# yellofi/SelectiveNet_for_semantic_segmentation_binary

Hardware: AMD Instinct MI355X
Metric: train images/sec, SelectiveUNet_B 256x256 bs=128 (global), selective_loss s_lamb=2 (higher is better)
Workload: dtype f32; 1 GPU; SelectiveUNet_B train step, global bs=128, 256x256, Adam lr=1e-3, s_lamb=2; model=SelectiveUNet_B, global_batch=128, per_gpu_batch=128, image=256, parallelism=dp1

## Files before the change

### include/selunet.h

```cpp
#ifndef SELUNET_H
#define SELUNET_H

#include <stdint.h>

#ifdef __cplusplus
extern "C" {
#endif

enum { SELUNET_F32 = 0, SELUNET_BF16 = 1 };

enum {
  SELUNET_OK = 0,
  SELUNET_EINVAL = 1,
  SELUNET_ELAUNCH = 2,
};

enum {
  SELUNET_OPT_HALO = 0,
  SELUNET_OPT_HALO_PERSIST,
  SELUNET_OPT_WINO,
  SELUNET_OPT_WINO_WGRAD,
  SELUNET_OPT_WINO_WGRAD_TW,
  SELUNET_OPT_WINO_WGRAD_WAVES,
  SELUNET_OPT_WGRAD_WGS,
  SELUNET_OPT_X2_WGRAD_WGS,
  SELUNET_OPT_GEMM_WGRAD_WGS,
  SELUNET_OPT_GATHER_WGS,
  SELUNET_OPT_RF_SINGLE,
  SELUNET_OPT_APPLY_U8,
  SELUNET_OPT_APPLY_GRID,
  SELUNET_OPT_X2D,
  SELUNET_OPT_TILE_QUEUE,
  SELUNET_OPT_X2P,
  SELUNET_OPT_CONVT_RING,
  SELUNET_OPT_COUNT
};
int64_t selunet_set_option(int32_t key, int64_t value);

#define SELUNET_GEMM_BM 128

typedef struct selunet_source {
  const void* data;
  const float* scale;
  const float* shift;
  int32_t channels;
  int32_t relu;
  int32_t layout;
  int32_t reserved;
} selunet_source;

typedef struct selunet_gather {
  int32_t n, h, w;
  int32_t taps;
  int32_t nsrc;
  int32_t reserved;
  selunet_source src[2];
} selunet_gather;

enum { SELUNET_EP_PLAIN = 0, SELUNET_EP_SPLIT = 1, SELUNET_EP_SCATTER2X = 2 };

typedef struct selunet_bn_bwd_stats {
  const void* y;
  const float* scale;
  const float* shift;
  const float* mean;
  const float* invstd;
  float* slab;
  float* amax;
} selunet_bn_bwd_stats;

typedef struct selunet_epilogue {
  void* out0;
  void* out1;
  const float* bias;
  float* stats;
  int32_t mode;
  int32_t split;
  float* colsum;
  selunet_bn_bwd_stats bnb;
  float* amax;
  const float* stats_center;
} selunet_epilogue;

const char* selunet_last_error(void);
int32_t selunet_version(void);
const char* selunet_build_id(void);

int selunet_pack_conv3x3(const float* w, int32_t co, int32_t ci, int32_t k_pad, void* fwd,
                         void* dgrad, int32_t dtype, void* stream);
int selunet_pack_convT(const float* w, int32_t ci, int32_t co, void* fwd, void* dgrad,
                       int32_t dtype, void* stream);
int selunet_unpack_conv3x3_grad(const float* packed, int32_t co, int32_t ci, int32_t k_pad,
                                float* out, void* stream);
int selunet_unpack_convT_grad(const float* packed, int32_t ci, int32_t co, float* out, void* stream);

int selunet_gemm_gather(const selunet_gather* a, const void* b, int32_t n_cols, int32_t k_pad,
                        const selunet_epilogue* ep, int32_t dtype, void* stream);
int32_t selunet_conv3x3_wino_ok(int32_t h, int32_t w, int32_t c_in, int32_t c_src0, int32_t n_cols);
int selunet_conv3x3_wino(const selunet_gather* a, const float* u, int32_t n_cols,
                         const selunet_epilogue* ep, void* stream);
const char* selunet_conv3x3_wino_kernel_name(int32_t n_cols, int32_t mode, int32_t split);
int selunet_gemm_gather_x2(const selunet_gather* a, const float* w, int32_t n_cols, int32_t k_pad,
                           const selunet_epilogue* ep, const float* amax0, const float* amax1, void* stream);
int64_t selunet_gemm_gather_x2_stats_rows(const selunet_gather* a, int32_t n_cols);
int64_t selunet_gemm_wgrad_x2_ws_bytes(const selunet_gather* p, const selunet_gather* q);
int selunet_gemm_wgrad_x2(const selunet_gather* p, const selunet_gather* q, float* ws, int64_t ws_bytes, int32_t layout,
                          float* out, const float* amax_p0, const float* amax_p1, const float* amax_q0,
                          const float* amax_q1, void* stream);
int32_t selunet_conv3x3_x2_ok(int32_t h, int32_t w, int32_t c_in, int32_t c_src0, int32_t n_cols);
int64_t selunet_conv3x3_wgrad_x2_ws_bytes(const selunet_gather* p, const selunet_gather* q);
int selunet_conv3x3_wgrad_x2(const selunet_gather* p, const selunet_gather* q, float* ws, int64_t ws_bytes,
                             float* out, const float* amax_p, const float* amax_q0, const float* amax_q1,
                             void* stream);
int selunet_conv3x3_wgrad_x2_bn(const selunet_gather* p, const selunet_gather* q, float* ws, int64_t ws_bytes,
                                float* out, const float* amax_p, const float* amax_q0, const float* amax_q1,
                                const selunet_bn_bwd_stats* bnb, const float* coef, float* dy, float* dy_amax,
                                void* stream);
enum { SELUNET_DA_TENSOR = 0, SELUNET_DA_POOL = 1, SELUNET_DA_HEADS = 2 };
typedef struct selunet_da_source {
  int32_t kind;
  int32_t nh;
  const float* pooled;
  const float* skip;
  const float* head_w;
  const float* g[3];
} selunet_da_source;
int selunet_conv3x3_wgrad_x2_bn_src(const selunet_gather* p, const selunet_gather* q, float* ws, int64_t ws_bytes,
                                    float* out, const float* amax_p, const float* amax_q0, const float* amax_q1,
                                    const selunet_bn_bwd_stats* bnb, const float* coef, const selunet_da_source* src,
                                    float* dy, float* dy_amax, void* stream);
int selunet_conv3x3_x2(const selunet_gather* a, const float* w, int32_t n_cols, const selunet_epilogue* ep,
                       const float* amax0, const float* amax1, void* stream);
const char* selunet_conv3x3_x2_kernel_name(const selunet_gather* a, int32_t n_cols, int32_t mode, int32_t split);
int64_t selunet_conv3x3_x2_stats_rows(const selunet_gather* a, int32_t n_cols);
int selunet_act_bound(const float* gamma, const float* beta, int32_t c, int64_t count, float* out, void* stream);
int selunet_act_amax(const float* y, int64_t m, int32_t c, const float* scale, const float* shift,
                     float* amax, void* stream);
int64_t selunet_gemm_stats_rows(const selunet_gather* a, int32_t n_cols, int32_t dtype);
int32_t selunet_set_halo_workgroups(int32_t wgs);
int32_t selunet_set_gather_workgroups(int32_t wgs);
const char* selunet_gemm_kernel_name(const selunet_gather* a, const selunet_gather* q, int32_t n_cols,
                                     int32_t mode, int32_t dtype);
int selunet_gemm_wgrad(const selunet_gather* p, const selunet_gather* q, float* out,
                       int32_t dtype, void* stream);
int64_t selunet_gemm_wgrad_ws_bytes(const selunet_gather* p, const selunet_gather* q, int32_t dtype);
int selunet_gemm_wgrad_ws(const selunet_gather* p, const selunet_gather* q, float* out, float* ws,
                          int64_t ws_bytes, int32_t dtype, void* stream);
int selunet_gemm_wgrad_ws_to(const selunet_gather* p, const selunet_gather* q, float* packed,
                             float* ws, int64_t ws_bytes, int32_t layout, float* out, int32_t dtype,
                             void* stream);
int32_t selunet_wgrad_ld(int32_t kq);

#define SELUNET_PACK_MAX 32
enum {
  SELUNET_PACK_CONV3X3 = 0,
  SELUNET_PACK_CONVT = 1,
  SELUNET_PACK_CONV3X3_WINO = 2,
  SELUNET_PACK_CONV3X3_X2 = 3,
  SELUNET_PACK_CONVT_X2 = 4,
  SELUNET_PACK_COPY = 5
};
typedef struct selunet_pack_desc {
  const float* w;
  void* fwd;
  void* dgrad;
  int32_t kind, co, ci, k_pad;
  int64_t offset;
} selunet_pack_desc;
typedef struct selunet_pack_list {
  int32_t n, _pad;
  selunet_pack_desc d[SELUNET_PACK_MAX];
} selunet_pack_list;
int selunet_pack_weights(const selunet_pack_list* list, int32_t dtype, void* stream);

int64_t selunet_reduce_ws_bytes(int32_t cols);
int selunet_reduce_rows(const float* slab, int64_t rows, int32_t cols, double* ws, double* out,
                        float* out32, void* stream);
int64_t selunet_channel_slab_rows(int64_t m);
int selunet_channel_sum(const void* x, int64_t m, int32_t c, float* slab, int32_t dtype, void* stream);

int selunet_bn_finalize(const double* sums, int64_t count, int32_t c, const float* conv_bias,
                        const float* gamma, const float* beta, float* running_mean,
                        float* running_var, int64_t* num_batches, float momentum, float eps,
                        int32_t training, float* mean, float* invstd, float* scale, float* shift,
                        void* stream);
int selunet_bn_bwd_reduce(const void* dz, const void* y, int64_t m, int32_t c, const float* scale,
                          const float* shift, const float* mean, const float* invstd, float* slab,
                          int32_t dtype, void* stream);
int selunet_bn_bwd_finalize(const double* sums, int64_t count, int32_t c, const float* gamma,
                            const float* invstd, float* dgamma, float* dbeta, float* dbias,
                            float* coef, void* stream);
int selunet_bn_stats_finalize(const float* slab, int64_t rows, double* ws, double* sums, int64_t count,
                              int32_t c, const float* conv_bias, const float* gamma, const float* beta,
                              float* running_mean, float* running_var, int64_t* num_batches,
                              float momentum, float eps, float* mean, float* invstd, float* scale,
                              float* shift, void* stream);
int64_t selunet_bn_centered_rows(int64_t m);
int selunet_bn_centered_partials(const void* y, int64_t m, int32_t c, const float* center, float* slab,
                                 int32_t dtype, void* stream);
int selunet_bn_centered_partials_adaptive(const void* y, int64_t m, int32_t c, const float* center,
                                          const float* uvar, float ratio, float* slab, int32_t dtype,
                                          void* stream);
int selunet_bn_stats_finalize_shifted(const float* slab, int64_t rows, double* ws, int64_t count, int32_t c,
                                      float* center, const float* conv_bias, const float* gamma,
                                      const float* beta, float ratio, float* mean, float* uvar_flag,
                                      float* invstd, float* scale, float* shift, void* stream);
int selunet_bn_stats_finalize_centered(const float* slab, int64_t rows, double* ws, double* sums,
                                       int64_t count, int32_t c, const float* center,
                                       const float* conv_bias, const float* gamma, const float* beta,
                                       float* running_mean, float* running_var, int64_t* num_batches,
                                       float momentum, float eps, float* mean, float* invstd,
                                       float* scale, float* shift, void* stream);
int selunet_bn_stats_finalize_centered_bound(const float* slab, int64_t rows, double* ws, double* sums,
// ... 204 lines not shown
```

### selectivenet_for_semantic_segmentation_binary_amd/_lib.py

```python
from __future__ import annotations

import ctypes
import os
import threading

import torch

from . import build as _build

c_int32, c_int64, c_double, c_float, c_void_p = (ctypes.c_int32, ctypes.c_int64, ctypes.c_double,
                                                ctypes.c_float, ctypes.c_void_p)

F32, BF16 = 0, 1
EP_PLAIN, EP_SPLIT, EP_SCATTER2X = 0, 1, 2
DA_TENSOR, DA_POOL, DA_HEADS = 0, 1, 2
GEMM_BM = 128
ADAM_CHUNK = 4096
SWEEP_MAX = 256
AUC_CHUNK = 4096


class Source(ctypes.Structure):
    _fields_ = [("data", c_void_p), ("scale", c_void_p), ("shift", c_void_p), ("channels", c_int32),
                ("relu", c_int32), ("layout", c_int32), ("reserved", c_int32)]


class Gather(ctypes.Structure):
    _fields_ = [("n", c_int32), ("h", c_int32), ("w", c_int32), ("taps", c_int32), ("nsrc", c_int32),
                ("reserved", c_int32), ("src", Source * 2)]


class BnBwdStats(ctypes.Structure):
    _fields_ = [("y", c_void_p), ("scale", c_void_p), ("shift", c_void_p), ("mean", c_void_p),
                ("invstd", c_void_p), ("slab", c_void_p), ("amax", c_void_p)]


class DaSource(ctypes.Structure):
    _fields_ = [("kind", c_int32), ("nh", c_int32), ("pooled", c_void_p), ("skip", c_void_p), ("head_w", c_void_p),
                ("g", c_void_p * 3)]


class Epilogue(ctypes.Structure):
    _fields_ = [("out0", c_void_p), ("out1", c_void_p), ("bias", c_void_p), ("stats", c_void_p),
                ("mode", c_int32), ("split", c_int32), ("colsum", c_void_p), ("bnb", BnBwdStats),
                ("amax", c_void_p), ("stats_center", c_void_p)]


class PackDesc(ctypes.Structure):
    _fields_ = [("w", c_void_p), ("fwd", c_void_p), ("dgrad", c_void_p), ("kind", c_int32), ("co", c_int32),
                ("ci", c_int32), ("k_pad", c_int32), ("offset", c_int64)]


PACK_MAX, PACK_CONV3X3, PACK_CONVT, PACK_CONV3X3_WINO, PACK_CONV3X3_X2, PACK_CONVT_X2, PACK_COPY = 32, 0, 1, 2, 3, 4, 5
WG_CONV3X3, WG_CONVT = 1, 2


class PackList(ctypes.Structure):
    _fields_ = [("n", c_int32), ("_pad", c_int32), ("d", PackDesc * PACK_MAX)]


class HeadPlanes(ctypes.Structure):
    _fields_ = [("n", c_int32), ("hw", c_int32), ("plane", c_void_p * 8), ("img_stride", c_int64 * 8),
                ("w_off", c_int32 * 8), ("b_off", c_int32 * 8), ("row_len", c_int32)]


class AdamTensor(ctypes.Structure):
    _fields_ = [("param", c_void_p), ("grad", c_void_p), ("exp_avg", c_void_p), ("exp_avg_sq", c_void_p),
                ("numel", c_int64), ("chunk_begin", c_int64)]


P = c_void_p
SIGNATURES = {
    "selunet_last_error": (ctypes.c_char_p, []),
    "selunet_version": (c_int32, []),
    "selunet_build_id": (ctypes.c_char_p, []),
    "selunet_pack_conv3x3": (c_int32, [P, c_int32, c_int32, c_int32, P, P, c_int32, P]),
    "selunet_pack_convT": (c_int32, [P, c_int32, c_int32, P, P, c_int32, P]),
    "selunet_unpack_conv3x3_grad": (c_int32, [P, c_int32, c_int32, c_int32, P, P]),
    "selunet_unpack_convT_grad": (c_int32, [P, c_int32, c_int32, P, P]),
    "selunet_gemm_gather": (c_int32, [ctypes.POINTER(Gather), P, c_int32, c_int32, ctypes.POINTER(Epilogue),
                                      c_int32, P]),
    "selunet_gemm_wgrad": (c_int32, [ctypes.POINTER(Gather), ctypes.POINTER(Gather), P, c_int32, P]),
    "selunet_wgrad_ld": (c_int32, [c_int32]),
    "selunet_gemm_wgrad_ws_bytes": (c_int64, [ctypes.POINTER(Gather), ctypes.POINTER(Gather), c_int32]),
    "selunet_gemm_wgrad_ws": (c_int32, [ctypes.POINTER(Gather), ctypes.POINTER(Gather), P, P, c_int64, c_int32, P]),
    "selunet_gemm_wgrad_ws_to": (c_int32, [ctypes.POINTER(Gather), ctypes.POINTER(Gather), P, P, c_int64, c_int32, P,
                                           c_int32, P]),
    "selunet_conv3x3_wino_ok": (c_int32, [c_int32, c_int32, c_int32, c_int32, c_int32]),
    "selunet_conv3x3_wino": (c_int32, [ctypes.POINTER(Gather), P, c_int32, ctypes.POINTER(Epilogue), P]),
    "selunet_conv3x3_wino_kernel_name": (ctypes.c_char_p, [c_int32, c_int32, c_int32]),
    "selunet_conv3x3_x2_ok": (c_int32, [c_int32, c_int32, c_int32, c_int32, c_int32]),
    "selunet_gemm_gather_x2": (c_int32, [ctypes.POINTER(Gather), P, c_int32, c_int32, ctypes.POINTER(Epilogue), P, P,
                                         P]),
    "selunet_conv3x3_x2": (c_int32, [ctypes.POINTER(Gather), P, c_int32, ctypes.POINTER(Epilogue), P, P, P]),
    "selunet_conv3x3_x2_kernel_name": (ctypes.c_char_p, [ctypes.POINTER(Gather), c_int32, c_int32, c_int32]),
    "selunet_conv3x3_x2_stats_rows": (c_int64, [ctypes.POINTER(Gather), c_int32]),
    "selunet_act_bound": (c_int32, [P, P, c_int32, c_int64, P, P]),
    "selunet_act_amax": (c_int32, [P, c_int64, c_int32, P, P, P, P]),
    "selunet_conv3x3_wgrad_x2_ws_bytes": (c_int64, [ctypes.POINTER(Gather), ctypes.POINTER(Gather)]),
    "selunet_gemm_wgrad_x2_ws_bytes": (c_int64, [ctypes.POINTER(Gather), ctypes.POINTER(Gather)]),
    "selunet_gemm_wgrad_x2": (c_int32, [ctypes.POINTER(Gather), ctypes.POINTER(Gather), P, c_int64, c_int32, P, P, P,
                                        P, P, P]),
    "selunet_conv3x3_wgrad_x2": (c_int32, [ctypes.POINTER(Gather), ctypes.POINTER(Gather), P, c_int64, P, P, P, P,
                                           P]),
    "selunet_conv3x3_wgrad_x2_bn": (c_int32, [ctypes.POINTER(Gather), ctypes.POINTER(Gather), P, c_int64, P, P, P, P,
                                              ctypes.POINTER(BnBwdStats), P, P, P, P]),
    "selunet_conv3x3_wgrad_x2_bn_src": (c_int32, [ctypes.POINTER(Gather), ctypes.POINTER(Gather), P, c_int64, P, P, P,
                                                  P, ctypes.POINTER(BnBwdStats), P, ctypes.POINTER(DaSource), P, P,
                                                  P]),
    "selunet_gemm_stats_rows": (c_int64, [ctypes.POINTER(Gather), c_int32, c_int32]),
    "selunet_gemm_gather_x2_stats_rows": (c_int64, [ctypes.POINTER(Gather), c_int32]),
    "selunet_set_halo_workgroups": (c_int32, [c_int32]),
    "selunet_set_gather_workgroups": (c_int32, [c_int32]),
    "selunet_gemm_kernel_name": (ctypes.c_char_p, [ctypes.POINTER(Gather), ctypes.POINTER(Gather), c_int32, c_int32,
                                                   c_int32]),
    "selunet_reduce_ws_bytes": (c_int64, [c_int32]),
    "selunet_reduce_rows": (c_int32, [P, c_int64, c_int32, P, P, P, P]),
    "selunet_channel_slab_rows": (c_int64, [c_int64]),
    "selunet_bn_centered_rows": (c_int64, [c_int64]),
    "selunet_channel_sum": (c_int32, [P, c_int64, c_int32, P, c_int32, P]),
    "selunet_bn_finalize": (c_int32, [P, c_int64, c_int32, P, P, P, P, P, P, c_float, c_float, c_int32, P, P, P, P,
                                      P]),
    "selunet_bn_bwd_reduce": (c_int32, [P, P, c_int64, c_int32, P, P, P, P, P, c_int32, P]),
    "selunet_bn_bwd_finalize": (c_int32, [P, c_int64, c_int32, P, P, P, P, P, P, P]),
    "selunet_pack_weights": (c_int32, [ctypes.POINTER(PackList), c_int32, P]),
    "selunet_bn_stats_finalize": (c_int32, [P, c_int64, P, P, c_int64, c_int32, P, P, P, P, P, P, c_float, c_float,
                                            P, P, P, P, P]),
    "selunet_bn_centered_partials": (c_int32, [P, c_int64, c_int32, P, P, c_int32, P]),
    "selunet_bn_centered_partials_adaptive": (c_int32, [P, c_int64, c_int32, P, P, c_float, P, c_int32, P]),
    "selunet_bn_stats_finalize_centered": (c_int32, [P, c_int64, P, P, c_int64, c_int32, P, P, P, P, P, P, P,
                                                     c_float, c_float, P, P, P, P, P]),
    "selunet_bn_stats_finalize_centered_bound": (c_int32, [P, c_int64, P, P, c_int64, c_int32, P, P, P, P, P, P, P,
                                                           c_float, c_float, P, P, P, P, P, P]),
    "selunet_bn_bwd_stats_finalize": (c_int32, [P, c_int64, P, P, c_int64, c_int32, P, P, P, P, P, P, P]),
    "selunet_bn_bwd_stats_finalize_bound": (c_int32, [P, c_int64, P, P, c_int64, c_int32, P, P, P, P, P, P, P, P, P]),
    "selunet_bn_bwd_apply": (c_int32, [P, P, c_int64, c_int32, P, P, P, P, P, P, c_int32, P]),
    "selunet_bn_bwd_apply_amax": (c_int32, [P, P, c_int64, c_int32, P, P, P, P, P, P, P, c_int32, P]),
    "selunet_bn_bwd_apply_heads": (c_int32, [P, c_int64, P, P, P, P, P, P, c_int32, P, P, P, P, P, c_int32, P]),
    "selunet_bn_bwd_apply_heads_planes": (c_int32, [P, c_int64, P, P, P, P, P, P, ctypes.POINTER(HeadPlanes), P, P,
                                                    c_int32, P]),
    "selunet_bn_bwd_apply_pool": (c_int32, [P, c_int32, c_int32, c_int32, c_int32, P, P, P, P, P, P, P, P, P,
                                            c_int32, P]),
    "selunet_im2col3x3": (c_int32, [P, c_int32, c_int32, c_int32, c_int32, c_int32, P, c_int32, P]),
    "selunet_maxpool2_fwd": (c_int32, [P, c_int32, c_int32, c_int32, c_int32, P, P, P, c_int32, P]),
    "selunet_maxpool2_bwd": (c_int32, [P, c_int32, c_int32, c_int32, c_int32, P, P, P, P, P,
                                       ctypes.POINTER(BnBwdStats), c_int32, P]),
    "selunet_maxpool2_bwd_slab_rows": (c_int64, [c_int32, c_int32, c_int32, c_int32]),
    "selunet_first_conv_rows": (c_int64, [c_int32, c_int32, c_int32]),
    "selunet_first_conv_fwd": (c_int32, [P, c_int32, c_int32, c_int32, c_int32, P, P, P, c_int32, P]),
    "selunet_first_conv_fwd_centered": (c_int32, [P, c_int32, c_int32, c_int32, c_int32, P, P, P, P, c_int32, P]),
    "selunet_bn_stats_finalize_shifted": (c_int32, [P, c_int64, P, c_int64, c_int32, P, P, P, P, c_float, P, P, P, P,
                                                    P, P]),
    "selunet_first_conv_wgrad_rows": (c_int64, [c_int32, c_int32, c_int32]),
    "selunet_first_conv_wgrad": (c_int32, [P, c_int32, c_int32, c_int32, c_int32, P, P, c_int32, P]),
    "selunet_first_conv_wgrad_bn": (c_int32, [P, c_int32, c_int32, c_int32, c_int32, P, P, P, P, P, P, P, P, c_int32,
                                              P]),
    "selunet_heads_fwd": (c_int32, [P, c_int64, P, P, P, P, c_int32, P, P, P, c_int32, P]),
    "selunet_heads_bwd": (c_int32, [P, c_int64, P, P, P, c_int32, P, P, P, P, P, ctypes.POINTER(BnBwdStats),
                                    c_int32, P]),
    "selunet_heads_fwd_planes": (c_int32, [P, c_int64, P, P, P, P, ctypes.POINTER(HeadPlanes), c_int32, P]),
    "selunet_heads_bwd_planes": (c_int32, [P, c_int64, P, P, P, ctypes.POINTER(HeadPlanes), P, P,
                                           ctypes.POINTER(BnBwdStats), c_int32, P]),
    "selunet_ce_selective_partials": (c_int32, [P, P, P, c_int64, c_int32, c_int64, P, P]),
    "selunet_ce_selective_bwd": (c_int32, [P, P, P, c_int64, c_int32, c_int64, P, c_float, P, P, P, P, P]),
    "selunet_ce_selective_partials_hard": (c_int32, [P, P, P, c_int64, c_int32, c_int64, P, P]),
    "selunet_ce_selective_bwd_hard": (c_int32, [P, P, P, c_int64, c_int32, c_int64, P, P, P, P, P]),
    "selunet_ce_partials": (c_int32, [P, P, c_int64, c_int32, c_int64, P, P]),
    "selunet_ce_bwd": (c_int32, [P, P, c_int64, c_int32, c_int64, c_double, P, P, P]),
    "selunet_loss_slab_rows": (c_int64, [c_int64]),
    "selunet_selective_partials": (c_int32, [P, P, P, c_int64, P, P]),
    "selunet_selective_finalize": (c_int32, [P, c_double, c_float, c_float, P, P, P, P]),
    "selunet_selective_bwd": (c_int32, [P, P, P, c_int64, P, c_float, P, P, P, P, P]),
    "selunet_selective_partials_hard": (c_int32, [P, P, P, c_int64, P, P]),
    "selunet_selective_bwd_hard": (c_int32, [P, P, P, c_int64, P, P, P, P, P]),
    "selunet_bce_partials": (c_int32, [P, P, c_int64, P, P]),
    "selunet_bce_finalize": (c_int32, [P, c_double, P, P]),
    "selunet_bce_bwd": (c_int32, [P, P, c_int64, c_double, P, P, P]),
    "selunet_adam_step": (c_int32, [P, c_int32, c_int64, c_float, c_float, c_float, c_float, c_float, c_int64, P]),
    "selunet_memset": (c_int32, [P, c_int32, c_int64, P]),
    "selunet_memcpy": (c_int32, [P, P, c_int64, P]),
    "selunet_stream_create": (c_int32, [ctypes.POINTER(P)]),
    "selunet_stream_destroy": (c_int32, [P]),
    "selunet_graph_capture_begin": (c_int32, [P]),
    "selunet_graph_capture_end": (c_int32, [P, ctypes.POINTER(P)]),
    "selunet_graph_launch": (c_int32, [P, P]),
    "selunet_graph_destroy": (c_int32, [P]),
    "selunet_prep_batch": (c_int32, [P, P, P, c_int32, c_int32, c_int32, c_int32, P, P, P]),
    "selunet_prep_batch_mode": (c_int32, [P, P, P, c_int32, c_int32, c_int32, c_int32, P, P, P]),
    "selunet_seg_metrics": (c_int32, [P, P, P, c_int64, c_float, c_float, P, P]),
    "selunet_seg_metrics_sweep": (c_int32, [P, P, P, c_int64, c_float, P, c_int32, P, P]),
    "selunet_seg_metrics_rows": (c_int32, [P, P, P, c_int32, c_int64, c_float, c_float, P, P]),
    "selunet_patch_auc": (c_int32, [P, P, P, c_int32, c_int64, c_float, P, P]),
    "selunet_tile_gather": (c_int32, [P, c_int32, c_int32, P, c_int32, c_int32, c_int32, c_int32, P, P]),
    "selunet_tile_stitch": (c_int32, [P, P, P, c_int32, c_int32, c_int32, c_int32, c_int32, c_int32, c_int32, c_int32,
                                      c_float, c_float, P, P, P, P, P, P]),
    "selunet_tile_gather_flip": (c_int32, [P, c_int32, c_int32, P, c_int32, c_int32, c_int32, c_int32, c_int32, P, P]),
    "selunet_image_transpose": (c_int32, [P, c_int32, c_int32, P, P]),
    "selunet_tta_accumulate": (c_int32, [P, P, P] + [c_int32] * 9 + [c_float, c_float, P, P, P, P, P]),
    "selunet_tta_finalize": (c_int32, [P] * 8 + [c_int32] * 5 + [c_float, c_float] + [P] * 8),
    "selunet_regions_label": (c_int32, [P, c_int64, c_int32, c_int32, c_int32, c_int32, P, P, P, c_int32, P, c_int32,
                                        P]),
    "selunet_regions_stats": (c_int32, [P, c_int32, P, c_int64, P, c_int64, c_int32, c_int32, P, c_int32, c_int64, P,
                                        P]),
    "selunet_regions_apply": (c_int32, [P, c_int64, c_int32, c_int32, P, c_int32, P, c_int32, P, c_int64, P, P]),
    "selunet_tissue_plane": (c_int32, [P, c_int32, c_int32, c_int32, c_int32, P, c_int32, P]),
    "selunet_tile_tissue_counts": (c_int32, [P, c_int64, c_int32, c_int32, P, c_int32, c_int32, c_int32, c_int32, P, P]),
    "selunet_tissue_class_counts": (c_int32, [P, c_int64, P, c_int64, c_int32, c_int32, P, P]),
    "selunet_set_option": (c_int64, [c_int32, c_int64]),
    "selunet_cu_hold": (c_int32, [P, P, c_int64, c_int32, c_float, P]),
}

_lib = None
_lock = threading.Lock()


def lib_path() -> str:
    return os.environ.get("SELUNET_LIB", _build.LIB)


def load(auto_build: bool = False):
    global _lib
    if _lib is not None:
        return _lib
    with _lock:
        if _lib is not None:
            return _lib
        path = lib_path()
        tree = _build.source_fingerprint()
        own = "SELUNET_LIB" not in os.environ
        if auto_build and own and (not os.path.exists(path) or _build.lib_stamp(path) != _build.build_id(tree)):
            _build.build(verbose=False)
        if not os.path.exists(path):
            raise RuntimeError(
                f"{path} not found: the MI355X kernels are not built (run "
                "`python -m selectivenet_for_semantic_segmentation_binary_amd.build`). "
                "There is no CPU fallback.")
        L = ctypes.CDLL(path)
        L.selunet_build_id.restype = ctypes.c_char_p
        built_fp, built_arch = _build.parse_build_id(L.selunet_build_id().decode())
        if own and built_fp != tree:
            raise RuntimeError(
                f"{path} was built from other sources (build id {built_fp}, for {built_arch}; tree "
                f"{tree}): rebuild with `python -m selectivenet_for_semantic_segmentation_binary_amd.build`")
        for name, (res, args) in SIGNATURES.items():
            fn = getattr(L, name)
            fn.restype = res
            fn.argtypes = args
        _lib = L
        for env, key in ENV_OPTIONS.items():
            v = os.environ.get(env)
            if v is not None and v.strip().lstrip("-").isdigit():
                L.selunet_set_option(key, int(v))
        if os.environ.get("SELUNET_NO_HALO") == "1":
            L.selunet_set_option(OPT["HALO"], 0)
    return _lib


OPT = {name: i for i, name in enumerate([
    "HALO", "HALO_PERSIST", "WINO", "WINO_WGRAD", "WINO_WGRAD_TW", "WINO_WGRAD_WAVES", "WGRAD_WGS",
    "X2_WGRAD_WGS", "GEMM_WGRAD_WGS", "GATHER_WGS", "RF_SINGLE", "APPLY_U8", "APPLY_GRID", "X2D",
    "TILE_QUEUE", "X2P", "CONVT_RING"])}
ENV_OPTIONS = {f"SELUNET_{k}": v for k, v in OPT.items() if k != "HALO"}


def set_option(name: str, value: int) -> int:
    return int(load().selunet_set_option(OPT[name], int(value)))


class SelunetError(RuntimeError):
    pass


_HOOK = None


def set_call_hook(hook):
    global _HOOK
    _HOOK = hook


def call(name, *args):
    L = load()
    fn = getattr(L, name)
    if _REC is not None:
        _REC.record(name, fn, args)
    rc = fn(*args) if _HOOK is None else _HOOK(name, args, lambda: fn(*args))
    if rc != 0:
        raise SelunetError(f"{name}: {L.selunet_last_error().decode()}")
    return rc


class Slot:
    __slots__ = ("name", "offset")

    def __init__(self, name, offset):
        self.name, self.offset = name, offset


class Plan:

    MAX_GRAPHS = 4

    def __init__(self, slots):
        self._ranges = [(n, t.data_ptr(), t.data_ptr() + t.numel() * t.element_size()) for n, t in slots.items()
                        if t is not None]
        self.calls = []
        self.keep = []
        self.stream = stream_ptr()
        self._graphs = {}
        self._seen = set()
        self._graphable = graphs_enabled()

    def _slot(self, v):
        if isinstance(v, int) and v:
            for n, lo, hi in self._ranges:
                if lo <= v < hi:
                    return Slot(n, v - lo)
        return None

    def record(self, name, fn, args):
        args = list(args)
        pos = []
        for i, a in enumerate(args):
            if isinstance(a, ctypes.Structure):
                fields = _struct_slots(a, self._slot)
                if fields:
                    args[i] = _StructSlots(type(a).from_buffer_copy(a), fields)
                    pos.append(i)
                continue
            sl = self._slot(a)
            if sl is not None:
                args[i] = sl
                pos.append(i)
        self.calls.append((name, fn, tuple(args), tuple(pos)))

    def record_marker(self, tag):
        self.calls.append((None, None, tag, ()))

    def _bound(self, base):
        for name, fn, args, pos in self.calls:
            if pos:
                a = list(args)
                for i in pos:
                    a[i] = a[i].bind(base) if isinstance(a[i], _StructSlots) else base[a[i].name] + a[i].offset
# ... 241 lines not shown
```

### selectivenet_for_semantic_segmentation_binary_amd/csrc/conv3x3.hip

```cpp
#include <cstdlib>

#include "gemm_common.h"

namespace selunet {

constexpr int TH = 16, TW = 16;
constexpr int HHT = TH + 2, HWT = TW + 2;
constexpr int HPIX = HHT * HWT;
constexpr int HTHREADS = 512;
constexpr int A_ROUNDS = (HPIX * 8 + HTHREADS - 1) / HTHREADS;
constexpr int AROWB = 160;
__device__ __forceinline__ int halo_off(int hp, int cc) { return hp * AROWB + ((cc ^ ((hp / HWT) & 1)) << 4); }

template <typename T, int BN, bool ONE_CHUNK>
__global__ void __launch_bounds__(HTHREADS, ONE_CHUNK ? 2 : 1)
conv3x3_halo_kernel(GatherArg g, const T* __restrict__ B, int N, int k_pad, EpiArg ep, int n_tiles, int tiles_x,
                    int tiles_y) {
  constexpr int E = 16 / sizeof(T);
  constexpr int CK = 128 / sizeof(T);
  constexpr int WAVES_N = BN / 64;
  constexpr int WAVES_M = 8 / WAVES_N;
  constexpr int WPIX = (TH * TW) / WAVES_M;
  constexpr int MT = WPIX / 32;
  constexpr int NT = 2;
// ... 133 lines not shown
  b_store(rb_next, 0);
  rb_next = b_load(nsteps > 1 ? 1 : 0);
  __syncthreads();

  if constexpr (ONE_CHUNK) {
#pragma unroll
    for (int t = 0; t < 9; ++t) {
      BRegs rb_far = rb_next;
      if (t + 2 < 9) rb_far = b_load(t + 2);
      mma_step(0, t & 1, t);
      if (t + 1 < 9) b_store(rb_next, (t + 1) & 1);
      __syncthreads();
      rb_next = rb_far;
    }
  } else {
    uint4 ra[A_ROUNDS];
    for (int c = 0; c < nchunks; ++c) {
      const int cn = c + 1 < nchunks ? c + 1 : c;
      int cs = cn * CK;
      const bool s1 = g.nsrc > 1 && cs >= g.src[0].C;
      if (s1) cs -= g.src[0].C;
      const SrcArg sn = pick_src(g, s1 ? 1 : 0);
      float* ssc = Ss + ((c + 1) & 1) * CK;
      float* ssh = Ss + 2 * CK + ((c + 1) & 1) * CK;
      float coef = 0.0f;
#pragma unroll
      for (int t = 0; t < 9; ++t) {
        const int s = c * 9 + t;
        const BRegs rb_far = b_load(s + 2 < nsteps ? s + 2 : nsteps - 1);
        if (t == 0 && sn.scale && tid < 2 * CK) coef = tid < CK ? sn.scale[cs + tid] : sn.shift[cs + tid - CK];
        if (t < A_ROUNDS) {
          int hp, cc;
          a_slot(t, hp, cc);
          ra[t] = *a_ptr(cn, hp, cc);
        }
        mma_step(c & 1, s & 1, t);
        b_store(rb_next, (s + 1) & 1);
        if (t == 1 && sn.scale && tid < 2 * CK) (tid < CK ? ssc[tid] : ssh[tid - CK]) = coef;
        if (t >= AD && t - AD < A_ROUNDS) {
          const int r = t - AD;
          int hp, cc;
          if (a_slot(r, hp, cc)) {
            uint4 v = make_uint4(0, 0, 0, 0);
            if (a_inside(hp)) {
              v = ra[r];
              if (sn.scale) {
                T e[E];
                __builtin_memcpy(e, &v, 16);
#pragma unroll
                for (int j = 0; j < E; ++j) {
                  float f = to_f(e[j]) * ssc[cc * E + j] + ssh[cc * E + j];
                  if (sn.relu) f = fmaxf(f, 0.0f);
                  e[j] = from_f<T>(f);
                }
                __builtin_memcpy(&v, e, 16);
              }
            }
            *reinterpret_cast<uint4*>(As + ((c + 1) & 1) * HPIX * AROWB + halo_off(hp, cc)) = v;
          }
        }
        __syncthreads();
        rb_next = rb_far;
      }
    }
  }

  float* tile = reinterpret_cast<float*>(smem);
  acc_to_lds<MT, NT, BN>(tile, acc, wm * WPIX, wn * 64, lane);
  __syncthreads();
  auto dst = [&](int pix, int c) -> T* {
    const int y = y0 + pix / TW, x = x0 + pix % TW;
    if (y >= g.h || x >= g.w) return nullptr;
    const int64_t m = ((int64_t)img * g.h + y) * g.w + x;
    const int col = n0 + c;
    if (ep.mode == SELUNET_EP_SPLIT)
      return col < ep.split ? reinterpret_cast<T*>(ep.out0) + m * ep.split + col
                            : reinterpret_cast<T*>(ep.out1) + m * (N - ep.split) + (col - ep.split);
    return reinterpret_cast<T*>(ep.out0) + m * N + col;
  };
  auto bias_col = [&](int c) { return n0 + c; };
  lds_tile_store<T, TH * TW, BN, HTHREADS>(tile, tid, dst, ep.bias, bias_col, tile_stats(ep, ptile, n0, N));
}

template <typename T, int BN, bool X2, bool M16 = false, bool TQ = false>
__global__ void __launch_bounds__(HTHREADS, 1)
conv3x3_halo_persist_kernel(GatherArg g, const T* __restrict__ B, int N, int k_pad, EpiArg ep, int n_tiles,
                            int tiles_x, int tiles_y, int ptiles, int gp, const float* __restrict__ wcs,
                            const float* __restrict__ amax0, const float* __restrict__ amax1,
                            unsigned* __restrict__ tq = nullptr) {
  static_assert(!TQ || X2, "tile queue: split-fp16 kernel only");
  static_assert(!X2 || std::is_same<T, float>::value, "split-fp16 form of fp32 operands only");
  static_assert(!M16 || X2, "16x16x32 form: split-fp16 only (the bf16 form lost every A/B, retired in round 6)");
  constexpr int E = 16 / sizeof(T);
  constexpr int CK = 128 / sizeof(T);
  constexpr int WAVES_N = BN / 64;
  constexpr int WAVES_M = 8 / WAVES_N;
  constexpr int WPIX = (TH * TW) / WAVES_M;
  constexpr int MT = WPIX / 32;
  constexpr int NT = 2;
  constexpr int RT = WPIX / 16;
  using AccT = std::conditional_t<M16, f32x4, f32x16>;
  constexpr int AM = M16 ? RT : MT, AN = M16 ? 4 : NT;
  constexpr int WROWB = M16 ? 160 : ROWB;
  constexpr int B_ROUNDS = BN * 8 / HTHREADS;
  static_assert(B_ROUNDS * HTHREADS == BN * 8, "weight tile rows must split evenly over the threads");
  auto halo_load_tap = [](int r) { return r; };
  auto halo_write_tap = [](int r) { return r + 3; };
  static_assert(A_ROUNDS <= 6, "halo slice schedule covers six slices");

  constexpr int SMEM_MAIN = 2 * HPIX * AROWB + 2 * BN * WROWB + 2 * CK * 8;
  constexpr int SMEM_EPI = TH * TW * (BN + 4) * 4;
  __shared__ __attribute__((aligned(16))) unsigned char smem[SMEM_MAIN > SMEM_EPI ? SMEM_MAIN : SMEM_EPI];
  unsigned char* As = smem;
  unsigned char* Bs = smem + 2 * HPIX * AROWB;
  float* Ss = reinterpret_cast<float*>(Bs + 2 * BN * WROWB);

  const int tid = threadIdx.x;
  const int lane = tid & 63, wave = tid >> 6;
  const int wm = wave / WAVES_N, wn = wave % WAVES_N;
  const int half = lane >> 5, l32 = lane & 31;
  const int l16 = lane & 15, kg = lane >> 4;

  const unsigned lb = xcd_remap(blockIdx.x, gridDim.x);
  const int n_tile = lb % n_tiles;
  const int prow = lb / n_tiles;
  const int n0 = n_tile * BN;
  const int nchunks = g.Ctot / CK;
  const int ntl = TQ ? 0 : (prow < ptiles ? (ptiles - prow + gp - 1) / gp : 0);
  __shared__ int tq_slot;
  int pt_cur = 0, pt_next = 0;
  if constexpr (TQ) {
    if (tid == 0) tq_slot = (int)min(atomicAdd(tq + n_tile, 1u), (unsigned)ptiles);
    __syncthreads();
    pt_cur = tq_slot;
  }
  const int csteps = nchunks * 9;
  float xs = 1.0f;
  float cfac[AN] = {};
  if constexpr (X2) {
    float am = amax0 ? amax0[0] : 0.0f;
    if (g.nsrc > 1 && amax1) am = fmaxf(am, amax1[0]);
    float inv;
    xs = x2_scale(am, &inv);
#pragma unroll
    for (int b = 0; b < AN; ++b)
      cfac[b] = wcs[n0 + wn * 64 + (M16 ? b * 16 + l16 : b * 32 + l32)] * inv;
  }
  auto halo_store = [&](int hb, int hp, int cc, uint4 v) __attribute__((always_inline)) {
    unsigned char* base = As + hb * HPIX * AROWB + hp * AROWB;
    if constexpr (X2) {
      float f[4];
      __builtin_memcpy(f, &v, 16);
      f16x4 h, l;
#pragma unroll
      for (int e = 0; e < 4; ++e) {
        _Float16 a, b;
        x2_split(f[e] * xs, a, b);
        h[e] = a;
        l[e] = b;
      }
      const int par = (hp / HWT) & 1;
      *reinterpret_cast<f16x4*>(base + (((cc >> 1) ^ par) << 4) + (cc & 1) * 8) = h;
      *reinterpret_cast<f16x4*>(base + (((4 + (cc >> 1)) ^ par) << 4) + (cc & 1) * 8) = l;
    } else {
      *reinterpret_cast<uint4*>(base + (((cc ^ ((hp / HWT) & 1))) << 4)) = v;
    }
  };

  auto halo_store_prepped = [&](int hb, int hp, int cc, uint4 v) __attribute__((always_inline)) {
    unsigned char* base = As + hb * HPIX * AROWB + hp * AROWB;
    if constexpr (X2) {
      const int par = (hp / HWT) & 1;
      *reinterpret_cast<uint2*>(base + (((cc >> 1) ^ par) << 4) + (cc & 1) * 8) = make_uint2(v.x, v.y);
      *reinterpret_cast<uint2*>(base + (((4 + (cc >> 1)) ^ par) << 4) + (cc & 1) * 8) = make_uint2(v.z, v.w);
// ... 368 lines not shown
            if (!defer) x_put((J + 1) & 1, r, xlds, o);
            else ra[r] = o;
            continue;
          }
          int hp, cc;
          if (a_slot(r, hp, cc)) {
            uint4 v = make_uint4(0, 0, 0, 0);
            if (a_inside(ny0, nx0, hp)) {
              v = ra[r];
              if (sn.scale) {
                T e[E];
                __builtin_memcpy(e, &v, 16);
#pragma unroll
                for (int j = 0; j < E; ++j) {
                  float f = to_f(e[j]) * ssc[cc * E + j] + ssh[cc * E + j];
                  if (sn.relu) f = fmaxf(f, 0.0f);
                  e[j] = from_f<T>(f);
                }
                __builtin_memcpy(&v, e, 16);
              }
            }
            if (!defer) {
              halo_store((J + 1) & 1, hp, cc, v);
            } else {
              if constexpr (X2) {
                float f[4];
                __builtin_memcpy(f, &v, 16);
                f16x4 h, l;
#pragma unroll
                for (int e = 0; e < 4; ++e) {
                  _Float16 a, b;
                  x2_split(f[e] * xs, a, b);
                  h[e] = a;
                  l[e] = b;
                }
                __builtin_memcpy(&v.x, &h, 8);
                __builtin_memcpy(&v.z, &l, 8);
              }
              ra[r] = v;
            }
          }
        }
        __syncthreads();
        rb_next = rb_far;
        ++S;
      }
      if (defer) {
      }
    }

    if constexpr (X2) {
#pragma unroll
      for (int a = 0; a < AM; ++a)
#pragma unroll
        for (int b = 0; b < AN; ++b) acc[a][b] *= cfac[b];
    }
    if constexpr (M16) {
#pragma unroll
      for (int a = 0; a < RT; ++a)
#pragma unroll
        for (int b = 0; b < 4; ++b)
#pragma unroll
          for (int i = 0; i < 4; ++i)
            tile[(wm * WPIX + a * 16 + 4 * kg + i) * (BN + 4) + wn * 64 + b * 16 + l16] = acc[a][b][i];
    } else {
      acc_to_lds<MT, NT, BN>(tile, acc, wm * WPIX, wn * 64, lane);
    }
#pragma unroll
    for (int a = 0; a < AM; ++a)
#pragma unroll
      for (int b = 0; b < AN; ++b) acc[a][b] = AccT{};
    __syncthreads();
    auto dst = [&](int pix, int cl) -> T* {
      const int y = y0 + pix / TW, x = x0 + pix % TW;
      if (y >= g.h || x >= g.w) return nullptr;
      const int64_t m = ((int64_t)img * g.h + y) * g.w + x;
      const int col = n0 + cl;
      if (ep.mode == SELUNET_EP_SPLIT)
        return col < ep.split ? reinterpret_cast<T*>(ep.out0) + m * ep.split + col
                              : reinterpret_cast<T*>(ep.out1) + m * (N - ep.split) + (col - ep.split);
      return reinterpret_cast<T*>(ep.out0) + m * N + col;
    };
    auto bias_col = [&](int cl) { return n0 + cl; };
    if constexpr (TQ) {
      TileStats tt = tile_stats(ep, pt_cur, n0, N);
      lds_tile_store_acc<T, TH * TW, BN, HTHREADS>(tile, tid, dst, ep.bias, bias_col, tt, s1, s2, s3, amx);
      tt.amax = nullptr;
      tile_stats_flush<BN, HTHREADS>(tile, tid, tt, s1, s2, s3, 0.0f);
#pragma unroll
      for (int e = 0; e < 8; ++e) s1[e] = s2[e] = s3[e] = 0;
    } else {
      lds_tile_store_acc<T, TH * TW, BN, HTHREADS>(tile, tid, dst, ep.bias, bias_col, ts, s1, s2, s3, amx);
    }
    if (TQ ? pt_next < ptiles : i + 1 < ntl) {
      __syncthreads();
      int tid2 = tid;
      asm volatile("" : "+v"(tid2));
#pragma unroll
      for (int r = 0; r < A_ROUNDS; ++r) {
        if constexpr (X2) {
          x_put(J & 1, r, x_lds(tid2), ra[r]);
        } else {
          const int hidx = r * HTHREADS + tid2;
          if (hidx < HPIX * 8) halo_store_prepped(J & 1, hidx >> 3, hidx & 7, ra[r]);
        }
      }
      b_store(rb_hold, S & 1);
      __syncthreads();
    }
    if constexpr (TQ) pt_cur = pt_next;
    gc = gn;
  }
  if constexpr (TQ) {
    if (ts.amax) block_amax(ts.amax, amx, tile);
    if (tid == 0 && atomicAdd(tq + n_tiles + n_tile, 1u) == (unsigned)gp - 1u) {
      atomicExch(tq + n_tile, 0u);
      atomicExch(tq + n_tiles + n_tile, 0u);
    }
  } else {
    tile_stats_flush<BN, HTHREADS>(tile, tid, ts, s1, s2, s3, amx);
  }
}

constexpr int WINO_STEPS = 12;
__device__ __forceinline__ int wino_row(int hp) {
  const int hy = hp / HWT, hx = hp - hy * HWT;
  return hy * HWT + (hx & 1) * (HWT / 2) + (hx >> 1);
}

template <int BN, int XS>
__global__ void __launch_bounds__(HTHREADS, 1)
conv3x3_wino_persist_kernel(GatherArg g, const float* __restrict__ B, int N, int k_pad, EpiArg ep, int n_tiles,
                            int tiles_x, int tiles_y, int ptiles, int gp) {
  using T = float;
  constexpr int E = 4;
  constexpr int CK = 32;
  constexpr int NT = BN / 64;
  constexpr int STEPS = WINO_STEPS / XS;
  constexpr int BROWS = XS * BN;
  constexpr int B_ROUNDS = BROWS * 8 / HTHREADS;
  static_assert(XS == 1 || XS == 2, "one or two planes per step");
  auto lt = [](int r) { return XS == 1 ? r : r >> 1; };
  static_assert(B_ROUNDS * HTHREADS == BROWS * 8, "weight tile rows must split evenly over the threads");
  static_assert(A_ROUNDS <= 6, "halo slice schedule covers six slices");

  constexpr int SMEM_MAIN = 2 * HPIX * AROWB + 2 * BROWS * ROWB + 2 * CK * 8;
  constexpr int SMEM_EPI = TH * TW * (BN + 4) * 4;
  __shared__ __attribute__((aligned(16))) unsigned char smem[SMEM_MAIN > SMEM_EPI ? SMEM_MAIN : SMEM_EPI];
  unsigned char* As = smem;
  unsigned char* Bs = smem + 2 * HPIX * AROWB;
  float* Ss = reinterpret_cast<float*>(Bs + 2 * BROWS * ROWB);

  const int tid = threadIdx.x;
  const int lane = tid & 63, wave = tid >> 6;
  const int wm = wave >> 1, wn = wave & 1;
  const int half = lane >> 5, l32 = lane & 31;
  const int pair = wm * 32 + l32, py = pair >> 3, px2 = pair & 7;

  const unsigned lb = xcd_remap(blockIdx.x, gridDim.x);
  const int n_tile = lb % n_tiles;
  const int prow = lb / n_tiles;
  const int n0 = n_tile * BN;
  const int ntl = prow < ptiles ? (ptiles - prow + gp - 1) / gp : 0;
  const int nchunks = g.Ctot / CK;
  const int csteps = nchunks * STEPS;

  auto tile_xy = [&](int i, int& img, int& y0, int& x0) __attribute__((always_inline)) {
    const unsigned pt = (unsigned)(prow + i * gp);
    const unsigned r = pt / (unsigned)tiles_x;
    x0 = (int)(pt - r * (unsigned)tiles_x) * TW;
    const unsigned r2 = r / (unsigned)tiles_y;
    y0 = (int)(r - r2 * (unsigned)tiles_y) * TH;
    img = (int)r2;
  };
  auto a_slot = [&](int round, int& hp, int& cc) -> bool {
// ... 1518 lines not shown
}

template <int BN, int XS>
static void launch_wino(const GatherArg& g, const float* u, int N, const EpiArg& ep, hipStream_t st) {
  const int tiles_x = (int)cdiv(g.w, TW), tiles_y = (int)cdiv(g.h, TH);
  const int n_tiles = N / BN;
  const int gp = persist_rows(g, N);
  hipLaunchKernelGGL((conv3x3_wino_persist_kernel<BN, XS>), dim3((unsigned)(gp * n_tiles)), dim3(HTHREADS), 0, st, g, u,
                     N, WINO_STEPS * g.Ctot, ep, n_tiles, tiles_x, tiles_y, (int)conv3x3_halo_tiles(g), gp);
}

bool conv3x3_bn128(int N, const EpiArg& ep, int split_mult) {
  return N % 128 == 0 && !(ep.mode == SELUNET_EP_SPLIT && ep.split % split_mult != 0);
}

int conv3x3_wino_launch(const GatherArg& g, const float* u, int N, const EpiArg& ep, hipStream_t st) {
  if (conv3x3_bn128(N, ep, 128)) launch_wino<128, 1>(g, u, N, ep, st);
  else launch_wino<64, 2>(g, u, N, ep, st);
  return check_launch("conv3x3_wino");
}

bool conv3x3_x2_shape_ok(int h, int w, int c_in, int c_src0, int n_cols) {
  return persist_enabled() && h >= TH && w >= TW && c_in % 32 == 0 && c_src0 % 32 == 0 && c_in > 32 &&
         n_cols % 64 == 0;
}

bool conv3x3_x2_eligible(const GatherArg& g, int N) {
  return conv3x3_halo_eligible(g, N, SELUNET_F32) && conv3x3_halo_persistent(g, SELUNET_F32) &&
         conv3x3_x2_shape_ok(g.h, g.w, g.Ctot, g.src[0].C, N);
}

bool x2_tile_queue() { return (option(SELUNET_OPT_TILE_QUEUE, 0) & 1) != 0; }

static unsigned* g_tq[64] = {};

int x2_tile_queue_prepare() {
  int dev = 0;
  if (hipGetDevice(&dev) != hipSuccess || dev < 0 || dev >= 64) return -1;
  if (g_tq[dev] != nullptr) return 0;
  unsigned* p = nullptr;
  if (hipMalloc(&p, 128 * sizeof(unsigned)) != hipSuccess) return -1;
  if (hipMemset(p, 0, 128 * sizeof(unsigned)) != hipSuccess || hipDeviceSynchronize() != hipSuccess) {
    (void)hipFree(p);
    return -1;
  }
  g_tq[dev] = p;
  return 0;
}

static unsigned* tq_counters(hipStream_t st) {
  int dev = 0;
  if (hipGetDevice(&dev) != hipSuccess || dev < 0 || dev >= 64) return nullptr;
  if (g_tq[dev] == nullptr) {
    hipStreamCaptureStatus cs = hipStreamCaptureStatusNone;
    if (hipStreamIsCapturing(st, &cs) != hipSuccess || cs != hipStreamCaptureStatusNone) return nullptr;
    if (x2_tile_queue_prepare() != 0) return nullptr;
  }
  return g_tq[dev];
}

int64_t conv3x3_x2_persist_rows(const GatherArg& g, int N) {
  if (conv3x3_x2p_eligible(g, N)) return conv3x3_x2p_rows(g, N);
  return x2_tile_queue() ? conv3x3_halo_tiles(g) : persist_rows(g, N);
}

template <int BN>
static int launch_x2(const GatherArg& g, const float* w, int N, const EpiArg& ep, const float* amax0,
                     const float* amax1, hipStream_t st) {
  const int tiles_x = (int)cdiv(g.w, TW), tiles_y = (int)cdiv(g.h, TH);
  const int n_tiles = N / BN;
  const int gp = persist_rows(g, N);
  const int k_pad = 9 * g.Ctot;
  const int cmax = std::max(g.src[0].C, g.nsrc > 1 ? g.src[1].C : 0);
  if (((int64_t)N * k_pad + N) * 4 >= (int64_t)1 << 31 || (int64_t)(HHT * g.w + HWT) * cmax * 4 >= (int64_t)1 << 31 ||
      (int64_t)3 * g.w + HWT >= 1 << 24 || (int64_t)cmax * 4 >= 1 << 24)
    return fail(SELUNET_EINVAL, "conv3x3_x2: operand too large for 32-bit staging offsets");
  unsigned* tq = nullptr;
  if (x2_tile_queue()) {
    tq = tq_counters(st);
    if (tq == nullptr || n_tiles > 64)
      return fail(SELUNET_ELAUNCH, "conv3x3_x2: tile-queue counters unavailable (set SELUNET_OPT_TILE_QUEUE "
                                   "before capturing the step)");
  }
  auto k = tq ? conv3x3_halo_persist_kernel<float, BN, true, BN == 64, true>
              : conv3x3_halo_persist_kernel<float, BN, true, BN == 64>;
  hipLaunchKernelGGL(k, dim3((unsigned)(gp * n_tiles)), dim3(HTHREADS), 0, st, g, w, N, k_pad, ep, n_tiles, tiles_x,
                     tiles_y, (int)conv3x3_halo_tiles(g), gp, w + (int64_t)N * k_pad, amax0, amax1, tq);
  return 0;
}

int conv3x3_x2_launch(const GatherArg& g, const float* w, int N, const EpiArg& ep, const float* amax0,
                      const float* amax1, hipStream_t st) {
  if (conv3x3_x2d_eligible(g, N)) return conv3x3_x2d_launch(g, w, ep, amax0, amax1, st);
  if (conv3x3_x2p_eligible(g, N)) return conv3x3_x2p_launch(g, w, N, ep, amax0, amax1, st);
  if (int rc = conv3x3_bn128(N, ep, 8) ? launch_x2<128>(g, w, N, ep, amax0, amax1, st)
                                       : launch_x2<64>(g, w, N, ep, amax0, amax1, st))
    return rc;
  return check_launch("conv3x3_x2");
}

int conv3x3_halo_launch(const GatherArg& g, const void* b, int N, int k_pad, const EpiArg& ep, int dtype,
                        hipStream_t st) {
  const bool one = halo_one_chunk(g, dtype);
  const bool bn128 = !one && conv3x3_bn128(N, ep, 128);
  if (dtype == SELUNET_F32) {
    if (bn128) launch_halo<float, 128>(g, b, N, k_pad, ep, st);
    else launch_halo<float, 64>(g, b, N, k_pad, ep, st);
  } else {
    if (bn128) launch_halo<__bf16, 128>(g, b, N, k_pad, ep, st);
    else launch_halo<__bf16, 64>(g, b, N, k_pad, ep, st);
  }
  return check_launch("conv3x3_halo");
}

}

extern "C" int32_t selunet_set_halo_workgroups(int32_t wgs) {
  const int prev = selunet::PERSIST_WGS;
  selunet::PERSIST_WGS = wgs > 0 ? wgs : selunet::PERSIST_WGS_DEFAULT;
  return prev;
}
```

### selectivenet_for_semantic_segmentation_binary_amd/csrc/conv3x3_x2d.hip

```cpp
#include "gemm_common.h"

namespace selunet {

constexpr int XD_TH = 16, XD_TW = 16, XD_HW = 18, XD_HPIX = 324;
constexpr int XD_THREADS = 256;
constexpr int XD_BN = 64;
constexpr int XD_CK = 32;
constexpr int XD_AROWB = 160;
constexpr int XD_WROWB = 160;
constexpr int XD_A_ROUNDS = (XD_HPIX * 8 + XD_THREADS - 1) / XD_THREADS;
constexpr int XD_B_ROUNDS = XD_BN * 8 / XD_THREADS;

__global__ void __launch_bounds__(XD_THREADS, 2)
conv3x3_x2d_kernel(GatherArg g, const float* __restrict__ B, int k_pad, EpiArg ep, int tiles_x, int tiles_y,
                   int ptiles, int gp, const float* __restrict__ wcs, const float* __restrict__ amax0,
                   const float* __restrict__ amax1) {
  constexpr int N = XD_BN;
  constexpr int OFF_B = XD_HPIX * XD_AROWB;
  constexpr int OFF_S = OFF_B + 2 * XD_BN * XD_WROWB;
  constexpr int SMEM_EPI = XD_TH * XD_TW * (XD_BN + 4) * 4;
  static_assert(SMEM_EPI <= OFF_S, "the epilogue tile must leave the coefficients alone");
  using Acc = double;
  static_assert(stats_flush_bytes<XD_BN, XD_THREADS, Acc>() <= OFF_S, "statistics scratch exceeds the tile");
  __shared__ __attribute__((aligned(16))) unsigned char smem[OFF_S + 2 * 2 * XD_CK * 4];
  unsigned char* As = smem;
  unsigned char* Bs = smem + OFF_B;
  float* Ss = reinterpret_cast<float*>(smem + OFF_S);

  const int tid = threadIdx.x;
  const int lane = tid & 63, wave = tid >> 6;
  const int l16 = lane & 15, kg = lane >> 4;

  const unsigned lb = xcd_remap(blockIdx.x, gridDim.x);
  const int prow = (int)lb;
  const int ntl = prow < ptiles ? (ptiles - prow + gp - 1) / gp : 0;
  const int nchunks = g.Ctot / XD_CK;
  const int csteps = nchunks * 9;
  const int njobs = ntl * nchunks;

  float xs, inv;
  {
    float am = amax0 ? amax0[0] : 0.0f;
    if (g.nsrc > 1 && amax1) am = fmaxf(am, amax1[0]);
    xs = x2_scale(am, &inv);
  }
  float cfac[4];
#pragma unroll
  for (int b = 0; b < 4; ++b) cfac[b] = wcs[b * 16 + l16] * inv;

  const int sq = tid >> 3, scc = tid & 7;
  const int say = sq >> 4, sax = sq & 15, sby = sq >> 1, sbx = 16 + (sq & 1);
  auto lds_of = [](int hy, int hx, int cc) __attribute__((always_inline)) {
    return (unsigned)((hy * XD_HW + hx) * XD_AROWB + (cc & 1) * 8 + (((cc >> 1) ^ (hy & 1)) << 4));
  };
  unsigned tb = 0;
  {
    const int hrem = g.h - (tiles_y - 1) * XD_TH, wrem = g.w - (tiles_x - 1) * XD_TW;
#pragma unroll
    for (int r = 0; r < XD_A_ROUNDS; ++r) {
      const int hy = r < 9 ? 2 * r + say : (r == 9 ? sby : 16 + sby);
      tb |= (unsigned)((hy == 0) | (hy > hrem) << 11) << r;
    }
    tb |= (unsigned)(sax == 0) << 22 | (unsigned)(sax > wrem) << 23 | (unsigned)(sbx > wrem) << 24 |
          (unsigned)(tid >= 32) << 25;
  }
  struct Geo {
    int img, y0, x0;
    int64_t pix;
    unsigned em;
  };
  auto tile_geo = [&](int i) __attribute__((always_inline)) {
    const unsigned pt = (unsigned)__builtin_amdgcn_readfirstlane(prow + i * gp);
    const unsigned r = pt / (unsigned)tiles_x, tx = pt - r * (unsigned)tiles_x;
    const unsigned r2 = r / (unsigned)tiles_y, ty = r - r2 * (unsigned)tiles_y;
    Geo q;
    q.img = (int)r2;
    q.y0 = (int)ty * XD_TH;
    q.x0 = (int)tx * XD_TW;
    const int64_t pix = ((int64_t)r2 * g.h + ty * XD_TH) * g.w + tx * XD_TW;
    q.pix = (int64_t)(((uint64_t)(unsigned)__builtin_amdgcn_readfirstlane((int)(pix >> 32)) << 32) |
                      (unsigned)__builtin_amdgcn_readfirstlane((int)pix));
    q.em = (unsigned)__builtin_amdgcn_readfirstlane(
        (int)((ty == 0 ? 0x7ffu : 0u) | (ty == (unsigned)tiles_y - 1u ? 0x7ffu << 11 : 0u) | (tx == 0 ? 1u << 22 : 0u) |
              (tx == (unsigned)tiles_x - 1u ? 3u << 23 : 0u) | 1u << 25));
    return q;
  };
  struct XStage {
    int64_t e0;
    unsigned oa, ob, stride_a, stride_b, safe, out;
  };
  auto x_stage = [&](const Geo& q, const SrcArg& sa, int c) __attribute__((always_inline)) {
    XStage s;
    s.e0 = (q.pix - g.w - 1) * sa.C + c;
    int tq = tid;
    asm volatile("" : "+v"(tq));
// ... 139 lines not shown
        sc[e] = sa.scale[c0 + (tid & 7) * 4 + e];
        sh[e] = sa.shift[c0 + (tid & 7) * 4 + e];
      }
    }
    a_split(ra, s0, sa.scale != nullptr, sc, sh, sa.relu);
    a_store(ra);
  }
  b_store(b_load(0), 0);
  BRegs rb_next = b_load(1 % csteps);
  __syncthreads();

  Acc s1[8] = {0, 0, 0, 0, 0, 0, 0, 0}, s2[8] = {0, 0, 0, 0, 0, 0, 0, 0}, s3[8] = {0, 0, 0, 0, 0, 0, 0, 0};
  float amx = 0.0f;
  const TileStats ts = tile_stats(ep, prow, 0, N);
  float* tile = reinterpret_cast<float*>(smem);
  float creg = 0.0f;
  int J = 0, S = 0;
  for (int i = 0; i < ntl; ++i) {
    const int img = gc.img, y0 = gc.y0, x0 = gc.x0;
    gn = i + 1 < ntl ? tile_geo(i + 1) : gc;
#pragma unroll
    for (int a = 0; a < 4; ++a)
#pragma unroll
      for (int b = 0; b < 4; ++b) acc[a][b] = f32x4{};
    BRegs rb_hold;
    for (int c = 0; c < nchunks; ++c, ++J) {
      const bool has_next = J + 1 < njobs;
      const bool last_c = c + 1 == nchunks;
      int cn;
      const SrcArg sn = chunk_src(last_c ? 0 : c + 1, cn);
      const XStage sx = x_stage(last_c ? gn : gc, sn, cn);
      float* ssn = Ss + ((J + 1) & 1) * 2 * XD_CK;
#pragma unroll
      for (int t = 0; t < 9; ++t) {
        const int st2 = c * 9 + t + 2;
        const BRegs rb_far = b_load(st2 < csteps ? st2 : st2 - csteps);
        if (has_next) {
          if (t == 0 && tid < 2 * XD_CK && sn.scale) creg = tid < XD_CK ? sn.scale[cn + tid] : sn.shift[cn + tid - XD_CK];
          if (t < (XD_A_ROUNDS + 1) / 2) a_load(ra, sx, sn, 2 * t, 2 * t + 2);
        }
        mma_tap(S & 1, t);
        if (t == 1 && has_next && tid < 2 * XD_CK) ssn[tid] = creg;
        if (t == 8 && has_next) {
          float sc[4] = {1, 1, 1, 1}, sh[4] = {0, 0, 0, 0};
          if (sn.scale) {
#pragma unroll
            for (int e = 0; e < 4; ++e) {
              sc[e] = ssn[(tid & 7) * 4 + e];
              sh[e] = ssn[XD_CK + (tid & 7) * 4 + e];
            }
          }
          a_split(ra, sx, sn.scale != nullptr, sc, sh, sn.relu);
        }
        if (last_c && has_next && t == 8) rb_hold = rb_next;
        else b_store(rb_next, (S + 1) & 1);
        __syncthreads();
        rb_next = rb_far;
        ++S;
      }
      if (!last_c) {
        a_store(ra);
        __syncthreads();
      }
    }

#pragma unroll
    for (int a = 0; a < 4; ++a)
#pragma unroll
      for (int b = 0; b < 4; ++b)
#pragma unroll
        for (int e = 0; e < 4; ++e)
          tile[((wave * 4 + a) * 16 + 4 * kg + e) * (N + 4) + b * 16 + l16] = acc[a][b][e] * cfac[b];
    __syncthreads();
    auto dst = [&](int pix, int cl) -> float* {
      const int y = y0 + pix / XD_TW, x = x0 + pix % XD_TW;
      if (y >= g.h || x >= g.w) return nullptr;
      const int64_t m = ((int64_t)img * g.h + y) * g.w + x;
      if (ep.mode == SELUNET_EP_SPLIT)
        return cl < ep.split ? reinterpret_cast<float*>(ep.out0) + m * ep.split + cl
                             : reinterpret_cast<float*>(ep.out1) + m * (N - ep.split) + (cl - ep.split);
      return reinterpret_cast<float*>(ep.out0) + m * N + cl;
    };
    auto bias_col = [&](int cl) { return cl; };
    lds_tile_store_acc<float, XD_TH * XD_TW, N, XD_THREADS>(tile, tid, dst, ep.bias, bias_col, ts, s1, s2, s3, amx);
    if (i + 1 < ntl) {
      __syncthreads();
      a_store(ra);
      b_store(rb_hold, S & 1);
      __syncthreads();
    }
    gc = gn;
  }
  tile_stats_flush<N, XD_THREADS>(tile, tid, ts, s1, s2, s3, amx);
}

int64_t conv3x3_x2d_rows(const GatherArg& g) {
  const int64_t pt = (int64_t)g.n * cdiv(g.h, XD_TH) * cdiv(g.w, XD_TW);
  return std::max<int64_t>(1, std::min<int64_t>(pt, 2 * (int64_t)conv3x3_persist_wgs()));
}

bool conv3x3_x2d_eligible(const GatherArg& g, int N) {
  const int64_t mode = option(SELUNET_OPT_X2D, 3);
  if (N != XD_BN || g.Ctot % XD_CK != 0 || mode <= 0) return false;
  if (mode == 1) return g.Ctot <= 1024;
  return g.Ctot <= 64 && (mode == 2 || g.src[0].scale != nullptr);
}

int conv3x3_x2d_launch(const GatherArg& g, const float* w, const EpiArg& ep, const float* amax0, const float* amax1,
                       hipStream_t st) {
  const int tiles_x = (int)cdiv(g.w, XD_TW), tiles_y = (int)cdiv(g.h, XD_TH);
  const int ptiles = (int)((int64_t)g.n * tiles_x * tiles_y);
  const int gp = (int)conv3x3_x2d_rows(g);
  const int k_pad = 9 * g.Ctot;
  const int cmax = std::max(g.src[0].C, g.nsrc > 1 ? g.src[1].C : 0);
  if (((int64_t)XD_BN * k_pad + XD_BN) * 4 >= (int64_t)1 << 31 ||
      (int64_t)((XD_TH + 2) * g.w + XD_HW) * cmax * 4 >= (int64_t)1 << 31 || (int64_t)16 * g.w + XD_HW >= 1 << 24 ||
      (int64_t)cmax * 4 >= 1 << 24 || (int64_t)k_pad * 4 >= 1 << 24)
    return fail(SELUNET_EINVAL, "conv3x3_x2d: operand too large for 32-bit staging offsets");
  hipLaunchKernelGGL(conv3x3_x2d_kernel, dim3((unsigned)gp), dim3(XD_THREADS), 0, st, g, w, k_pad, ep, tiles_x, tiles_y,
                     ptiles, gp, w + (int64_t)XD_BN * k_pad, amax0, amax1);
  return check_launch("conv3x3_x2d");
}

}
```

### selectivenet_for_semantic_segmentation_binary_amd/csrc/gemm.hip

```cpp
#include <type_traits>

#include "gemm_common.h"

namespace selunet {

template <typename T, int BN, bool SMALL, bool X2, int BMT = BM, int NTH = 256>
__global__ void __launch_bounds__(NTH, NTH == 256 ? 2 : 1)
gemm_gather_kernel(GatherArg g, const T* __restrict__ B, int N, int k_pad, EpiArg ep, int n_tiles, int P,
                   const float* __restrict__ wcs, const float* __restrict__ amax0, const float* __restrict__ amax1) {
  static_assert(!X2 || (std::is_same<T, float>::value && !SMALL), "split-fp16 form: fp32 vector gathers");
  constexpr int E = 16 / sizeof(T);
  constexpr int BKE = 128 / sizeof(T);
  constexpr int WN = BN / 2;
  constexpr int NT = WN / 32;
  constexpr int MT = 2;
  constexpr int RP = NTH / 8;
  constexpr int AR = BMT / RP;
  constexpr int BR = BN / RP;
  static_assert(BMT == 64 * (NTH / 64) / 2, "two wave columns of 64-row waves");

  constexpr int SMEM_MAIN = 2 * (BMT + BN) * ROWB, SMEM_EPI = BMT * (BN + 4) * 4 + BMT * 8;
  __shared__ __attribute__((aligned(16))) unsigned char smem[SMEM_MAIN > SMEM_EPI ? SMEM_MAIN : SMEM_EPI];
  unsigned char* As = smem;
  unsigned char* Bs = smem + 2 * BMT * ROWB;
// ... 883 lines not shown
  const int n_tiles = N / BN;
  const int64_t P = gather_rows(g, N);
  hipLaunchKernelGGL((gemm_gather_kernel<T, BN, SMALL, false>), dim3((unsigned)(P * n_tiles)), dim3(256), 0, st, g,
                     reinterpret_cast<const T*>(b), N, k_pad, ep, n_tiles, (int)P, nullptr, nullptr, nullptr);
}

template <typename T, int BI, int BJ>
static void launch_wgrad(const GatherArg& p, const GatherArg& q, float* out, int ldo, int ni, int nj_pad,
                         hipStream_t st, float* ws = nullptr) {
  if (p.small || q.small) launch_wgrad_impl<T, BI, BJ, true>(p, q, out, ldo, ni, nj_pad, ws, st);
  else launch_wgrad_impl<T, BI, BJ, false>(p, q, out, ldo, ni, nj_pad, ws, st);
}

template <typename T, int BI, int BJ, bool SMALL>
static void launch_wgrad_impl(const GatherArg& p, const GatherArg& q, float* out, int ldo, int ni, int nj_pad,
                              float* ws, hipStream_t st) {
  const int tiles_j = nj_pad / BJ;
  const int tiles = (ni / BI) * tiles_j;
  int64_t mchunk;
  const int64_t splits = wgrad_splits(p.M, tiles, &mchunk);
  if constexpr (std::is_same<T, float>::value)
    hipLaunchKernelGGL((gemm_wgrad_kernel<T, BI, BJ, SMALL>), dim3((unsigned)(tiles * splits)), dim3(256), 0, st, p, q, out,
                       ldo, mchunk, tiles_j, tiles, ws, (int64_t)ni * ldo);
  else
    hipLaunchKernelGGL((gemm_wgrad_bf16_kernel<BI, BJ, SMALL>), dim3((unsigned)(tiles * splits)), dim3(256), 0, st, p, q,
                       out, ldo, mchunk, tiles_j, tiles, ws, (int64_t)ni * ldo);
}

}

using namespace selunet;

bool selunet::halo_enabled() { return option(SELUNET_OPT_HALO, 1) != 0; }

extern "C" int32_t selunet_set_gather_workgroups(int32_t wgs) {
  const int32_t prev = (int32_t)selunet::gather_wgs();
  g_options[SELUNET_OPT_GATHER_WGS] = wgs < 0 ? -1 : wgs;
  return prev;
}

extern "C" int64_t selunet_gemm_stats_rows(const selunet_gather* a, int32_t n_cols, int32_t dtype) {
  const int esz = dtype == SELUNET_F32 ? 4 : 2;
  GatherArg g;
  if (make_gather(a, dtype, g, 16 / esz)) return -1;
  if (halo_enabled() && conv3x3_halo_eligible(g, n_cols, dtype)) return conv3x3_halo_stats_rows(g, n_cols, dtype);
  if (dtype == SELUNET_BF16 && convt_ring_bf16_dgrad_operand_ok(g, n_cols)) return convt_ring_rows(g, n_cols);
  if (dtype == SELUNET_BF16 && convt_dgrad_bf16_ntb(g, n_cols) > 0) return convt_dgrad_bf16_rows(g, n_cols);
  return gather_rows(g, n_cols);
}

extern "C" const char* selunet_gemm_kernel_name(const selunet_gather* a, const selunet_gather* q, int32_t n_cols,
                                                int32_t mode, int32_t dtype) {
  const bool bf = dtype == SELUNET_BF16;
  const int esz = bf ? 2 : 4;
  GatherArg g;
  if (q == nullptr) {
    if (make_gather(a, dtype, g, 16 / esz)) return "invalid";
    if (mode != SELUNET_EP_SCATTER2X && halo_enabled() && conv3x3_halo_eligible(g, n_cols, dtype)) {
      const bool one = conv3x3_halo_one_chunk(g, dtype);
      const bool bn128 = !one && n_cols % 128 == 0 && !(mode == SELUNET_EP_SPLIT && (n_cols / 2) % 128 != 0);
      if (one) return bf ? "conv3x3_halo1<bf16,64>" : "conv3x3_halo1<f32,64>";
      if (conv3x3_halo_persistent(g, dtype))
        return bf ? (bn128 ? "conv3x3_halo_persist<bf16,128>" : "conv3x3_halo_persist<bf16,64>")
                  : (bn128 ? "conv3x3_halo_persist<f32,128>" : "conv3x3_halo_persist<f32,64>");
      return bf ? (bn128 ? "conv3x3_halo<bf16,128>" : "conv3x3_halo<bf16,64>")
                : (bn128 ? "conv3x3_halo<f32,128>" : "conv3x3_halo<f32,64>");
    }
    if (bf && mode == SELUNET_EP_SCATTER2X && convt_bf16_fwd_ntb(g, n_cols) > 0) return "convt<bf16>";
    if (bf && mode == SELUNET_EP_PLAIN && convt_dgrad_bf16_ntb(g, n_cols) > 0) return "convt_dgrad<bf16>";
    return bf ? "gemm_gather<bf16>" : "gemm_gather<f32>";
  }
  GatherArg gq;
  const int vec = bf ? 8 : 4;
  if (make_gather(a, dtype, g, vec) || make_gather(q, dtype, gq, vec)) return "invalid";
  if (halo_enabled() && conv3x3_wgrad_wino_eligible(g, gq, dtype)) return "conv3x3_wgrad_wino_f32<64>";
  if (halo_enabled() && conv3x3_wgrad_halo_eligible(g, gq, dtype)) {
    if (bf) return g.K % 128 == 0 ? "conv3x3_wgrad_halo<128>" : "conv3x3_wgrad_halo<64>";
    return g.K % 128 == 0 ? "conv3x3_wgrad_halo_f32<128>" : "conv3x3_wgrad_halo_f32<64>";
  }
  return bf ? "gemm_wgrad_bf16" : "gemm_wgrad<f32>";
}

static int check_gather_call(const selunet_gather* a, const void* b, int32_t n_cols, int32_t k_pad,
                             const selunet_epilogue* ep, int32_t dtype, GatherArg& g, EpiArg& e) {
  SELUNET_REQUIRE(dtype == SELUNET_F32 || dtype == SELUNET_BF16, "dtype must be SELUNET_F32 or SELUNET_BF16");
  const int esz = dtype == SELUNET_F32 ? 4 : 2;
  const int bke = 128 / esz;
  if (int rc = make_gather(a, dtype, g, 16 / esz)) return rc;
  SELUNET_REQUIRE(b != nullptr && ep != nullptr && ep->out0 != nullptr, "B / epilogue / out0 must be non-NULL");
  SELUNET_REQUIRE(n_cols > 0 && n_cols % 64 == 0, "n_cols must be a positive multiple of 64 (got %d)", n_cols);
  SELUNET_REQUIRE(k_pad >= g.K && k_pad % bke == 0, "k_pad (%d) must be >= K (%d) and a multiple of %d", k_pad, g.K,
                  bke);
  SELUNET_REQUIRE(g.small || (g.Ctot % bke == 0 && (a->nsrc == 1 || a->src[0].channels % bke == 0)),
                  "vector gather needs channel counts that are multiples of %d", bke);
  SELUNET_REQUIRE(ep->mode >= 0 && ep->mode <= 2, "bad epilogue mode");
  if (ep->mode == SELUNET_EP_SPLIT)
    SELUNET_REQUIRE(ep->out1 != nullptr && ep->split > 0 && ep->split < n_cols && ep->split % 64 == 0,
                    "split epilogue needs out1 and 0 < split < n_cols, split %% 64 == 0");
  if (ep->mode == SELUNET_EP_SCATTER2X)
    SELUNET_REQUIRE(n_cols % 4 == 0 && a->taps == 1, "scatter2x epilogue needs taps == 1 and n_cols % 4 == 0");
  SELUNET_REQUIRE(ep->stats == nullptr || ep->mode == SELUNET_EP_PLAIN, "stats only with the plain epilogue");
  SELUNET_REQUIRE(ep->colsum == nullptr || ep->mode == SELUNET_EP_SPLIT, "colsum only with the split epilogue");
  const selunet_bn_bwd_stats& bb = ep->bnb;
  if (bb.slab != nullptr)
    SELUNET_REQUIRE(ep->mode == SELUNET_EP_PLAIN && ep->stats == nullptr && bb.y && bb.scale && bb.shift && bb.mean &&
                        bb.invstd && ep->bias == nullptr,
                    "bn-backward sums need the plain epilogue without stats/bias and y/scale/shift/mean/invstd");
  e = EpiArg{ep->out0, ep->out1, ep->bias, ep->stats, ep->mode, ep->split, ep->colsum,
             BnBwdArg{bb.y, bb.scale, bb.shift, bb.mean, bb.invstd, bb.slab}, ep->amax, ep->stats_center};
  SELUNET_REQUIRE(ep->stats_center == nullptr || ep->stats != nullptr, "stats_center only with stats");
  return SELUNET_OK;
}

extern "C" int selunet_gemm_gather(const selunet_gather* a, const void* b, int32_t n_cols, int32_t k_pad,
                                   const selunet_epilogue* ep, int32_t dtype, void* stream) {
  GatherArg g;
  EpiArg e;
  if (int rc = check_gather_call(a, b, n_cols, k_pad, ep, dtype, g, e)) return rc;
  hipStream_t st = as_stream(stream);
  if (ep->mode != SELUNET_EP_SCATTER2X && halo_enabled() && conv3x3_halo_eligible(g, n_cols, dtype))
    return conv3x3_halo_launch(g, b, n_cols, k_pad, e, dtype, st);
  if (dtype == SELUNET_BF16) {
    if (convt_ring_bf16_takes(g, n_cols, e)) return convt_ring_bf16_launch(g, b, n_cols, e, st);
    if (convt_bf16_eligible(g, n_cols, e) || convt_dgrad_bf16_eligible(g, n_cols, e))
      return convt_bf16_launch(g, b, n_cols, e, st);
    SELUNET_REQUIRE(convt_dgrad_bf16_ntb(g, n_cols) == 0 || (e.stats == nullptr && e.colsum == nullptr &&
                                                             e.bnb.slab == nullptr),
                    "gemm_gather: statistics epilogue on a ConvTranspose2d data-gradient operand that "
                    "selunet_gemm_stats_rows sizes for the resident-weight kernel (PLAIN, no amax / bias)");
  }
  const bool bn128 = n_cols % 128 == 0 && !(ep->mode == SELUNET_EP_SPLIT && ep->split % 128 != 0);
  if (dtype == SELUNET_F32) {
    if (bn128) launch_gather<float, 128>(g, b, n_cols, k_pad, e, st);
    else launch_gather<float, 64>(g, b, n_cols, k_pad, e, st);
  } else {
    if (bn128) launch_gather<__bf16, 128>(g, b, n_cols, k_pad, e, st);
    else launch_gather<__bf16, 64>(g, b, n_cols, k_pad, e, st);
  }
  return check_launch("gemm_gather");
}

extern "C" int32_t selunet_conv3x3_wino_ok(int32_t h, int32_t w, int32_t c_in, int32_t c_src0, int32_t n_cols) {
  return halo_enabled() && conv3x3_wino_shape_ok(h, w, c_in, c_src0, n_cols) ? 1 : 0;
}

extern "C" const char* selunet_conv3x3_wino_kernel_name(int32_t n_cols, int32_t mode, int32_t split) {
  EpiArg e{};
  e.mode = mode;
  e.split = split;
  return conv3x3_bn128(n_cols, e, 128) ? "conv3x3_wino<f32,128>" : "conv3x3_wino<f32,64>";
}

extern "C" int selunet_conv3x3_wino(const selunet_gather* a, const float* u, int32_t n_cols,
                                   const selunet_epilogue* ep, void* stream) {
  GatherArg g;
  EpiArg e;
  SELUNET_REQUIRE(a != nullptr && a->taps == 9, "conv3x3_wino: a 3x3 (taps = 9) gather is required");
  if (int rc = check_gather_call(a, u, n_cols, 12 * a->src[0].channels + 12 * (a->nsrc > 1 ? a->src[1].channels : 0),
                                 ep, SELUNET_F32, g, e))
    return rc;
  SELUNET_REQUIRE(ep->mode != SELUNET_EP_SCATTER2X, "conv3x3_wino: scatter epilogue not supported");
  SELUNET_REQUIRE(halo_enabled() && conv3x3_wino_eligible(g, n_cols),
                  "conv3x3_wino: operand not eligible (%dx%d, C=%d, n_cols=%d; see selunet_conv3x3_wino_ok)", g.h, g.w,
                  g.Ctot, n_cols);
  return conv3x3_wino_launch(g, u, n_cols, e, as_stream(stream));
}

constexpr int X2_BM = 256;

static int x2_bn(int n_cols, const EpiArg& e) {
  if (n_cols % 128 != 0 || (e.mode == SELUNET_EP_SPLIT && e.split % 128 != 0)) return 64;
  return 128;
}

static int64_t x2_rows(const GatherArg& g, int N) {
  if (convt_ring_dgrad_operand_ok(g, N)) return convt_ring_rows(g, N);
  if (convt_dgrad_x2_ntb(g, N) > 0) return convt_dgrad_x2_rows(g, N);
  if (N % 128 != 0) return gather_rows(g, N);
  const int64_t m_tiles = cdiv(g.M, X2_BM);
  const int64_t wgs = gather_wgs();
  if (wgs == 0) return m_tiles;
  return std::max<int64_t>(1, std::min<int64_t>(m_tiles, std::max<int64_t>(1, wgs / 2) / cdiv(N, 128)));
}

extern "C" int64_t selunet_gemm_gather_x2_stats_rows(const selunet_gather* a, int32_t n_cols) {
  GatherArg g;
  if (make_gather(a, SELUNET_F32, g, 4)) return -1;
  return x2_rows(g, n_cols);
}

extern "C" int selunet_gemm_gather_x2(const selunet_gather* a, const float* w, int32_t n_cols, int32_t k_pad,
                                      const selunet_epilogue* ep, const float* amax0, const float* amax1,
                                      void* stream) {
  GatherArg g;
  EpiArg e;
  if (int rc = check_gather_call(a, w, n_cols, k_pad, ep, SELUNET_F32, g, e)) return rc;
  SELUNET_REQUIRE(!g.small && k_pad == g.K && g.K % 32 == 0,
                  "gemm_gather_x2: vector gathers with K (%d) a multiple of 32 and k_pad == K", g.K);
  SELUNET_REQUIRE(amax0 != nullptr && (a->nsrc == 1 || amax1 != nullptr),
                  "gemm_gather_x2: every source needs its range word (amax0, amax1)");
  hipStream_t st = as_stream(stream);
  if (convt_ring_x2_takes(g, n_cols, e)) return convt_ring_x2_launch(g, w, n_cols, e, amax0, st);
  if (convt_x2_eligible(g, n_cols, e)) return convt_x2_launch(g, w, n_cols, e, amax0, st);
  if (convt_dgrad_x2_eligible(g, n_cols, e)) return convt_dgrad_x2_launch(g, w, n_cols, e, amax0, st);
  const int bn = x2_bn(n_cols, e);
  const int64_t P = x2_rows(g, n_cols);
  const float* wcs = w + (int64_t)n_cols * k_pad;
  const dim3 grid((unsigned)(P * (n_cols / bn)));
  if (bn == 128)
    hipLaunchKernelGGL((gemm_gather_kernel<float, 128, false, true, X2_BM, 512>), grid, dim3(512), 0, st, g, w,
                       n_cols, k_pad, e, n_cols / 128, (int)P, wcs, amax0, amax1);
  else
    hipLaunchKernelGGL((gemm_gather_kernel<float, 64, false, true>), grid, dim3(256), 0, st, g, w, n_cols, k_pad, e,
                       n_cols / 64, (int)P, wcs, amax0, amax1);
  return check_launch("gemm_gather_x2");
}

extern "C" int32_t selunet_conv3x3_x2_ok(int32_t h, int32_t w, int32_t c_in, int32_t c_src0, int32_t n_cols) {
  return halo_enabled() && conv3x3_x2_shape_ok(h, w, c_in, c_src0, n_cols) ? 1 : 0;
}

extern "C" const char* selunet_conv3x3_x2_kernel_name(const selunet_gather* a, int32_t n_cols, int32_t mode,
                                                      int32_t split) {
  EpiArg e{};
  e.mode = mode;
  e.split = split;
  GatherArg g;
  if (make_gather(a, SELUNET_F32, g, 4)) return "?";
  if (conv3x3_x2d_eligible(g, n_cols)) return "conv3x3_x2d<f32,64>";
  if (conv3x3_x2p_eligible(g, n_cols)) return "conv3x3_x2p<f32,128>";
  return conv3x3_bn128(n_cols, e, 8) ? "conv3x3_x2<f32,128>" : "conv3x3_x2<f32,64>";
}

extern "C" int64_t selunet_conv3x3_x2_stats_rows(const selunet_gather* a, int32_t n_cols) {
  GatherArg g;
  if (make_gather(a, SELUNET_F32, g, 4)) return -1;
  if (conv3x3_x2d_eligible(g, n_cols)) return conv3x3_x2d_rows(g);
  return conv3x3_x2_persist_rows(g, n_cols);
}

extern "C" int selunet_conv3x3_x2(const selunet_gather* a, const float* w, int32_t n_cols, const selunet_epilogue* ep,
                                  const float* amax0, const float* amax1, void* stream) {
  GatherArg g;
  EpiArg e;
  SELUNET_REQUIRE(a != nullptr && a->taps == 9, "conv3x3_x2: a 3x3 (taps = 9) gather is required");
  if (int rc = check_gather_call(a, w, n_cols, 9 * (a->src[0].channels + (a->nsrc > 1 ? a->src[1].channels : 0)), ep,
                                 SELUNET_F32, g, e))
    return rc;
  SELUNET_REQUIRE(ep->mode != SELUNET_EP_SCATTER2X, "conv3x3_x2: scatter epilogue not supported");
  SELUNET_REQUIRE(amax0 != nullptr && (a->nsrc == 1 || amax1 != nullptr),
                  "conv3x3_x2: every source needs its range word (amax0, amax1)");
  SELUNET_REQUIRE(halo_enabled() && conv3x3_x2_eligible(g, n_cols),
                  "conv3x3_x2: operand not eligible (%dx%d, C=%d, n_cols=%d; see selunet_conv3x3_x2_ok)", g.h, g.w,
                  g.Ctot, n_cols);
  return conv3x3_x2_launch(g, w, n_cols, e, amax0, amax1, as_stream(stream));
}

enum { WG_PACKED = 0, WG_CONV3X3 = 1, WG_CONVT = 2 };
template <int LAYOUT>
__global__ void __launch_bounds__(64) wgrad_reduce_kernel(const float* __restrict__ ws, int64_t splits,
                                                          int64_t stride, int ni, int ldo, int kq,
                                                          float* __restrict__ out) {
  constexpr int U = 16;
  const int64_t n4 = (int64_t)ni * ldo / 4;
  for (int64_t v = blockIdx.x * (int64_t)blockDim.x + threadIdx.x; v < n4; v += (int64_t)gridDim.x * blockDim.x) {
    const int64_t e = v * 4;
    const int j = (int)(e % ldo);
    f32x4 acc = {0, 0, 0, 0};
    if (j < kq) {
      int64_t sp = 0;
      for (; sp + U <= splits; sp += U) {
        f32x4 x[U];
#pragma unroll
        for (int u = 0; u < U; ++u) x[u] = *reinterpret_cast<const f32x4*>(ws + (sp + u) * stride + e);
#pragma unroll
        for (int u = 0; u < U; ++u) acc += x[u];
      }
      for (; sp < splits; ++sp) acc += *reinterpret_cast<const f32x4*>(ws + sp * stride + e);
      if (j + 4 > kq)
        for (int u = 0; u < 4; ++u)
          if (j + u >= kq) acc[u] = 0.0f;
    }
    if constexpr (LAYOUT == WG_PACKED) {
      *reinterpret_cast<f32x4*>(out + e) = acc;
    } else {
      const int64_t row = e / ldo;
#pragma unroll
      for (int u = 0; u < 4; ++u) {
        const int jj = j + u;
        if (jj >= kq) continue;
        if constexpr (LAYOUT == WG_CONV3X3) {
          const int ci = kq / 9, tap = jj / ci, c = jj - tap * ci;
          out[(row * ci + c) * 9 + tap] = acc[u];
        } else {
          const int co = kq / 4, ab = jj / co, o = jj - ab * co;
          out[(row * co + o) * 4 + ab] = acc[u];
        }
      }
    }
  }
}

template <int LAYOUT>
__global__ void __launch_bounds__(64) wgrad_wino_reduce_kernel(const float* __restrict__ ws, int64_t splits,
                                                               int64_t stride, int ni, int ctot, int ldo,
                                                               float* __restrict__ out) {
  const int c4n = ctot / 4;
  const int64_t n = (int64_t)ni * 3 * c4n;
  const int ldw = 12 * ctot;
  for (int64_t v = blockIdx.x * (int64_t)blockDim.x + threadIdx.x; v < n; v += (int64_t)gridDim.x * blockDim.x) {
    const int c = (int)(v % c4n) * 4;
    const int64_t r2 = v / c4n;
    const int dy = (int)(r2 % 3);
    const int64_t row = r2 / 3;
    const float* base = ws + row * ldw + dy * 4 * ctot + c;
    f32x4 m[4] = {{0, 0, 0, 0}, {0, 0, 0, 0}, {0, 0, 0, 0}, {0, 0, 0, 0}};
    constexpr int U = 4;
    int64_t sp = 0;
    for (; sp + U <= splits; sp += U) {
      f32x4 x[U][4];
#pragma unroll
      for (int u = 0; u < U; ++u)
#pragma unroll
        for (int k = 0; k < 4; ++k) x[u][k] = *reinterpret_cast<const f32x4*>(base + (sp + u) * stride + k * ctot);
#pragma unroll
      for (int u = 0; u < U; ++u)
#pragma unroll
        for (int k = 0; k < 4; ++k) m[k] += x[u][k];
    }
    for (; sp < splits; ++sp)
#pragma unroll
// ... 359 lines not shown
```

### selectivenet_for_semantic_segmentation_binary_amd/csrc/gemm_common.h

```cpp
#pragma once

#include <type_traits>

#include "common.h"

namespace selunet {

struct SrcArg {
  const void* data;
  const float* scale;
  const float* shift;
  int C;
  int relu;
  int layout;
  int pad;
};

struct GatherArg {
  int n, h, w;
  int taps;
  int nsrc;
  int Ctot;
  int hs, ws;
  int K;
// ... 56 lines not shown
template <typename T>
__device__ __forceinline__ float gather_scalar(const GatherArg& g, int64_t m, int k) {
  if (m >= g.M || k >= g.K) return 0.0f;
  const int tap = k / g.Ctot;
  int c = k - tap * g.Ctot;
  int s = 0;
  if (g.nsrc > 1 && c >= g.src[0].C) {
    c -= g.src[0].C;
    s = 1;
  }
  const int x = (int)(m % g.w);
  const int64_t t = m / g.w;
  const int y = (int)(t % g.h);
  const int img = (int)(t / g.h);
  int ys, xs;
  if (!src_pixel(g, tap, y, x, ys, xs)) return 0.0f;
  const SrcArg sa = pick_src(g, s);
  float v;
  if (sa.layout == 1) {
    v = reinterpret_cast<const float*>(sa.data)[(((int64_t)img * sa.C + c) * g.hs + ys) * g.ws + xs];
  } else {
    v = to_f(reinterpret_cast<const T*>(sa.data)[(((int64_t)img * g.hs + ys) * g.ws + xs) * sa.C + c]);
  }
  if (sa.scale) {
    v = v * sa.scale[c] + sa.shift[c];
    if (sa.relu) v = fmaxf(v, 0.0f);
  }
  return v;
}

template <typename T> struct Mma;
template <> struct Mma<float> {
  __device__ static inline void run(f32x16& acc, uint4 a, uint4 b) {
    acc = __builtin_amdgcn_mfma_f32_32x32x2f32(__uint_as_float(a.x), __uint_as_float(b.x), acc, 0, 0, 0);
    acc = __builtin_amdgcn_mfma_f32_32x32x2f32(__uint_as_float(a.y), __uint_as_float(b.y), acc, 0, 0, 0);
    acc = __builtin_amdgcn_mfma_f32_32x32x2f32(__uint_as_float(a.z), __uint_as_float(b.z), acc, 0, 0, 0);
    acc = __builtin_amdgcn_mfma_f32_32x32x2f32(__uint_as_float(a.w), __uint_as_float(b.w), acc, 0, 0, 0);
  }
};
template <> struct Mma<__bf16> {
  __device__ static inline void run(f32x16& acc, uint4 a, uint4 b) {
    bf16x8 av = __builtin_bit_cast(bf16x8, a);
    bf16x8 bv = __builtin_bit_cast(bf16x8, b);
    acc = __builtin_amdgcn_mfma_f32_32x32x16_bf16(av, bv, acc, 0, 0, 0);
  }
};

template <typename T>
__device__ __forceinline__ uint4 transform16(uint4 raw, const float* scale, const float* shift, int c, int relu) {
  constexpr int E = 16 / sizeof(T);
  T v[E];
  __builtin_memcpy(v, &raw, 16);
#pragma unroll
  for (int e = 0; e < E; ++e) {
    float f = to_f(v[e]) * scale[c + e] + shift[c + e];
    if (relu) f = fmaxf(f, 0.0f);
    v[e] = from_f<T>(f);
  }
  uint4 out;
  __builtin_memcpy(&out, v, 16);
  return out;
}

struct BnBwdArg {
  const void* y;
  const float* scale;
  const float* shift;
  const float* mean;
  const float* invstd;
  float* slab;
};

struct EpiArg {
  void* out0;
  void* out1;
  const float* bias;
  float* stats;
  int mode;
  int split;
  float* colsum;
  BnBwdArg bnb;
  float* amax;
  const float* stats_center;
};

typedef short s16x4 __attribute__((ext_vector_type(4)));

__device__ __forceinline__ unsigned xcd_remap(unsigned b, unsigned nb) {
  const unsigned xcd = b & 7u, q = nb >> 3, r = nb & 7u;
  const unsigned base = xcd < r ? xcd * (q + 1) : r * (q + 1) + (xcd - r) * q;
  return base + (b >> 3);
}

template <int MT, int NT, int TC>
__device__ __forceinline__ void acc_to_lds(float* tile, const f32x16 (&acc)[MT][NT], int wr0, int wc0, int lane) {
  const int half = lane >> 5, l32 = lane & 31;
#pragma unroll
  for (int a = 0; a < MT; ++a)
#pragma unroll
    for (int b = 0; b < NT; ++b)
#pragma unroll
      for (int r = 0; r < 16; ++r)
        tile[(wr0 + a * 32 + (r & 3) + 8 * (r >> 2) + 4 * half) * (TC + 4) + wc0 + b * 32 + l32] = acc[a][b][r];
}

struct TileStats {
  float* stats;
  int ld;
  float* colsum;
  int colsum_cols;
  int gcol0;
  BnBwdArg bnb;
  const void* out0;
  float* amax;
  const float* center;
};

__device__ __forceinline__ TileStats tile_stats(const EpiArg& ep, int64_t row, int n0, int N) {
  TileStats ts;
  ts.ld = N;
  ts.stats = ep.stats ? ep.stats + row * 2 * N + n0 : nullptr;
  ts.colsum = ep.colsum ? ep.colsum + row * ep.split + n0 : nullptr;
  ts.colsum_cols = ep.split;
  ts.gcol0 = n0;
  ts.bnb = ep.bnb;
  if (ep.bnb.slab) {
    ts.bnb.scale += n0;
    ts.bnb.shift += n0;
    ts.bnb.mean += n0;
    ts.bnb.invstd += n0;
    ts.bnb.slab += row * 3 * N + n0;
  }
  ts.out0 = ep.out0;
  ts.amax = ep.amax;
  ts.center = ep.stats_center ? ep.stats_center + n0 : nullptr;
  return ts;
}

template <typename T> struct StatAcc { using type = float; };
template <> struct StatAcc<float> { using type = double; };

template <typename T, int TR, int TC, int NTHREADS, typename Dst, typename BiasCol, typename Acc>
__device__ __forceinline__ void lds_tile_store_acc(float* tile, int tid, Dst&& dst, const float* bias,
                                                   BiasCol&& bias_col, const TileStats& ts, Acc (&s1)[8],
                                                   Acc (&s2)[8], Acc (&s3)[8], float& am) {
  constexpr int CC = TC / 8;
  constexpr int RS = NTHREADS / CC;
  asm volatile("" : "+v"(tid));
  const int cc = tid % CC, r0 = tid / CC;
  const int col = cc * 8;
  float bv[8], cen[8];
#pragma unroll
  for (int e = 0; e < 8; ++e) bv[e] = bias ? bias[bias_col(col + e)] : 0.0f;
  const bool do_st = ts.stats != nullptr;
#pragma unroll
  for (int e = 0; e < 8; ++e) cen[e] = do_st && ts.center ? ts.center[col + e] : 0.0f;
  const bool do_cs = ts.colsum != nullptr && ts.gcol0 + col < ts.colsum_cols;
  const bool do_bn = ts.bnb.slab != nullptr;
  float sc[8], sh[8], mu[8], is[8];
  if (do_bn) {
#pragma unroll
    for (int e = 0; e < 8; ++e) {
      sc[e] = ts.bnb.scale[col + e];
      sh[e] = ts.bnb.shift[col + e];
      mu[e] = ts.bnb.mean[col + e];
      is[e] = ts.bnb.invstd[col + e];
// ... 49 lines not shown
#pragma unroll
    for (int e = 0; e < 8; ++e) o[e] = from_f<T>(v[e]);
    if (ts.amax) {
#pragma unroll
      for (int e = 0; e < 8; ++e) am = fmaxf(am, fabsf(to_f(o[e])));
    }
    if constexpr (sizeof(T) == 2) {
      uint4 u;
      __builtin_memcpy(&u, o, 16);
      *reinterpret_cast<uint4*>(p) = u;
    } else {
      *reinterpret_cast<f32x4*>(p) = f32x4{v[0], v[1], v[2], v[3]};
      *reinterpret_cast<f32x4*>(p + 4) = f32x4{v[4], v[5], v[6], v[7]};
    }
    if (do_cs) {
#pragma unroll
      for (int e = 0; e < 8; ++e) t1[e] += to_f(o[e]);
    }
    if (do_bn) {
#pragma unroll
      for (int e = 0; e < 8; ++e) {
        const float y = to_f(yb[j][e]);
        const float da = y * sc[e] + sh[e] > 0.0f ? to_f(o[e]) : 0.0f;
        const float xh = (y - mu[e]) * is[e];
        t1[e] += da;
        t2[e] += da * xh;
        t3[e] += xh;
      }
    }
  }
  }
  if constexpr (WIDE) {
#pragma unroll
    for (int e = 0; e < 8; ++e) {
      s1[e] += (Acc)t1[e];
      s2[e] += (Acc)t2[e];
      s3[e] += (Acc)t3[e];
    }
  }
}

template <int TC, int NTHREADS, typename Acc>
constexpr int stats_flush_bytes() { return (NTHREADS / (TC / 8)) * TC * 3 * (int)sizeof(Acc); }

template <int TC, int NTHREADS, typename Acc>
__device__ __forceinline__ void tile_stats_flush(float* red_f, int tid, const TileStats& ts, const Acc (&s1)[8],
                                                 const Acc (&s2)[8], const Acc (&s3)[8], float am) {
  constexpr int CC = TC / 8;
  constexpr int RS = NTHREADS / CC;
  Acc* red = reinterpret_cast<Acc*>(red_f);
  const int cc = tid % CC, r0 = tid / CC;
  const int col = cc * 8;
  const bool do_st = ts.stats != nullptr;
  const bool do_bn = ts.bnb.slab != nullptr;
  const int nst = do_bn ? 3 : (do_st ? 2 : 1);
  if (do_st || ts.colsum != nullptr || do_bn) {
    __syncthreads();
#pragma unroll
    for (int e = 0; e < 8; ++e) {
      red[(r0 * TC + col + e) * 3 + 0] = s1[e];
      red[(r0 * TC + col + e) * 3 + 1] = s2[e];
      red[(r0 * TC + col + e) * 3 + 2] = s3[e];
    }
    __syncthreads();
    for (int i = tid; i < TC * nst; i += NTHREADS) {
      const int c = i % TC, k = i / TC;
      Acc a = 0;
      for (int r = 0; r < RS; ++r) a += red[(r * TC + c) * 3 + k];
      if (do_bn) ts.bnb.slab[k * ts.ld + c] = a;
      else if (do_st) ts.stats[k * ts.ld + c] = a;
      else if (ts.gcol0 + c < ts.colsum_cols) ts.colsum[c] = a;
    }
  }
  if (ts.amax) block_amax(ts.amax, am, red_f);
}

template <typename T, int TR, int TC, int NTHREADS, typename Dst, typename BiasCol>
__device__ __forceinline__ void lds_tile_store(float* tile, int tid, Dst&& dst, const float* bias, BiasCol&& bias_col,
                                               const TileStats& ts) {
  float s1[8] = {0, 0, 0, 0, 0, 0, 0, 0}, s2[8] = {0, 0, 0, 0, 0, 0, 0, 0}, s3[8] = {0, 0, 0, 0, 0, 0, 0, 0};
  float am = 0.0f;
  lds_tile_store_acc<T, TR, TC, NTHREADS>(tile, tid, dst, bias, bias_col, ts, s1, s2, s3, am);
  tile_stats_flush<TC, NTHREADS>(tile, tid, ts, s1, s2, s3, am);
}

int make_gather(const selunet_gather* a, int dtype, GatherArg& g, int vec_elems);

bool conv3x3_halo_eligible(const GatherArg& g, int N, int dtype);
int64_t conv3x3_halo_tiles(const GatherArg& g);
int64_t conv3x3_halo_stats_rows(const GatherArg& g, int N, int dtype);
bool conv3x3_halo_one_chunk(const GatherArg& g, int dtype);
bool conv3x3_halo_persistent(const GatherArg& g, int dtype);
int conv3x3_halo_launch(const GatherArg& g, const void* b, int N, int k_pad, const EpiArg& ep, int dtype,
                        hipStream_t st);
bool conv3x3_wino_shape_ok(int h, int w, int c_in, int c_src0, int n_cols);
bool conv3x3_wgrad_wino_eligible(const GatherArg& p, const GatherArg& q, int dtype);
int64_t conv3x3_wgrad_wino_splits(const GatherArg& p, const GatherArg& q);
int conv3x3_wgrad_wino_launch(const GatherArg& p, const GatherArg& q, float* ws, int ldw, hipStream_t st);
bool conv3x3_wino_eligible(const GatherArg& g, int N);
bool conv3x3_bn128(int N, const EpiArg& ep, int split_mult);
int conv3x3_wino_launch(const GatherArg& g, const float* u, int N, const EpiArg& ep, hipStream_t st);
bool conv3x3_x2_shape_ok(int h, int w, int c_in, int c_src0, int n_cols);
bool conv3x3_x2_eligible(const GatherArg& g, int N);
int conv3x3_x2_launch(const GatherArg& g, const float* w, int N, const EpiArg& ep, const float* amax0,
                      const float* amax1, hipStream_t st);
bool convt_x2_eligible(const GatherArg& g, int N, const EpiArg& e);
int convt_dgrad_x2_ntb(const GatherArg& g, int N);
int64_t convt_dgrad_x2_rows(const GatherArg& g, int N);
bool convt_dgrad_x2_eligible(const GatherArg& g, int N, const EpiArg& e);
int convt_dgrad_x2_launch(const GatherArg& g, const float* w, int N, const EpiArg& e, const float* amax_src,
                          hipStream_t st);
bool convt_ring_dgrad_operand_ok(const GatherArg& g, int N);
int64_t convt_ring_rows(const GatherArg& g, int N);
bool convt_ring_x2_takes(const GatherArg& g, int N, const EpiArg& e);
int convt_ring_x2_launch(const GatherArg& g, const float* w, int N, const EpiArg& e, const float* amax_src,
                         hipStream_t st);
bool convt_ring_bf16_dgrad_operand_ok(const GatherArg& g, int N);
bool convt_ring_bf16_takes(const GatherArg& g, int N, const EpiArg& e);
int convt_ring_bf16_launch(const GatherArg& g, const void* w, int N, const EpiArg& e, hipStream_t st);
int convt_bf16_fwd_ntb(const GatherArg& g, int N);
int convt_dgrad_bf16_ntb(const GatherArg& g, int N);
int64_t convt_dgrad_bf16_rows(const GatherArg& g, int N);
bool convt_bf16_eligible(const GatherArg& g, int N, const EpiArg& e);
bool convt_dgrad_bf16_eligible(const GatherArg& g, int N, const EpiArg& e);
int convt_bf16_launch(const GatherArg& g, const void* w, int N, const EpiArg& e, hipStream_t st);
int convt_x2_launch(const GatherArg& g, const float* w, int N, const EpiArg& e, const float* amax_src,
                    hipStream_t st);
int64_t conv3x3_persist_rows(const GatherArg& g, int N);
int conv3x3_persist_wgs();
bool conv3x3_x2d_eligible(const GatherArg& g, int N);
int64_t conv3x3_x2d_rows(const GatherArg& g);
int conv3x3_x2d_launch(const GatherArg& g, const float* w, const EpiArg& ep, const float* amax0, const float* amax1,
                       hipStream_t st);
bool conv3x3_wgrad_halo_eligible(const GatherArg& p, const GatherArg& q, int dtype);
int64_t conv3x3_wgrad_x2_splits(const GatherArg& p, const GatherArg& q);
bool x2_tile_queue();
bool conv3x3_x2p_eligible(const GatherArg& g, int N);
int64_t conv3x3_x2p_rows(const GatherArg& g, int N);
int conv3x3_x2p_launch(const GatherArg& g, const float* w, int N, const EpiArg& ep, const float* amax0,
                       const float* amax1, hipStream_t st);
int64_t conv3x3_x2_persist_rows(const GatherArg& g, int N);
struct WgradBnArg {
  const float* y;
  const float* scale;
  const float* shift;
  const float* mean;
  const float* invstd;
  const float* coef;
  float* dy;
  float* dy_amax;
  int kind;
  int nh;
  const float* pooled;
  const float* skip;
  const float* hw;
  const float* g0;
  const float* g1;
  const float* g2;
};
int conv3x3_wgrad_x2_launch(const GatherArg& p, const GatherArg& q, float* ws, int ldo, const float* amax_p,
                            const float* amax_q0, const float* amax_q1, hipStream_t st,
                            const WgradBnArg* bn = nullptr);
int conv3x3_wgrad_halo_launch(const GatherArg& p, const GatherArg& q, float* out, int ldo, float* ws, int dtype,
                              hipStream_t st);
int64_t conv3x3_wgrad_halo_splits(const GatherArg& p, const GatherArg& q, int dtype);
bool halo_enabled();
// ... 3 lines not shown
```

### selectivenet_for_semantic_segmentation_binary_amd/csrc/pointwise.hip

```cpp
#include <cstdarg>
#include <cstdlib>
#include <cmath>

#include "common.h"

namespace selunet {

static thread_local char g_err[512] = "";

int64_t g_options[SELUNET_OPT_COUNT] = {-1, -1, -1, -1, -1, -1, -1, -1, -1, -1, -1, -1, -1, -1, -1, -1, -1};
static_assert(SELUNET_OPT_COUNT == 17, "g_options initialiser: one -1 per option");

void set_error(const char* fmt, ...) {
  va_list ap;
  va_start(ap, fmt);
  vsnprintf(g_err, sizeof(g_err), fmt, ap);
  va_end(ap);
}

int fail(int code, const char* fmt, ...) {
  va_list ap;
  va_start(ap, fmt);
  vsnprintf(g_err, sizeof(g_err), fmt, ap);
  va_end(ap);
  return code;
}

int check_launch(const char* what) {
  hipError_t e = hipGetLastError();
  if (e != hipSuccess) return fail(SELUNET_ELAUNCH, "%s: %s", what, hipGetErrorString(e));
  return SELUNET_OK;
}

constexpr int TPB = 256;

template <typename T>
__global__ void pack_conv3x3_kernel(const float* __restrict__ w, int co, int ci, int k_pad, T* fwd, T* dgrad) {
  const int64_t total_f = (int64_t)co * k_pad;
  const int64_t total_d = dgrad ? (int64_t)ci * 9 * co : 0;
  for (int64_t i = blockIdx.x * (int64_t)blockDim.x + threadIdx.x; i < total_f + total_d;
       i += (int64_t)gridDim.x * blockDim.x) {
    if (i < total_f) {
      const int o = (int)(i / k_pad), k = (int)(i % k_pad);
      float v = 0.0f;
      if (k < 9 * ci) {
        const int tap = k / ci, c = k - tap * ci;
        v = w[((int64_t)o * ci + c) * 9 + tap];
      }
      fwd[i] = from_f<T>(v);
    } else {
      const int64_t j = i - total_f;
      const int c = (int)(j / (9 * co));
      const int k = (int)(j % (9 * co));
      const int tap = k / co, o = k - tap * co;
      dgrad[j] = from_f<T>(w[((int64_t)o * ci + c) * 9 + (8 - tap)]);
    }
  }
}

template <typename T>
__global__ void pack_convT_kernel(const float* __restrict__ w, int ci, int co, T* fwd, T* dgrad) {
  const int64_t total = (int64_t)ci * co * 4;
  for (int64_t i = blockIdx.x * (int64_t)blockDim.x + threadIdx.x; i < total; i += (int64_t)gridDim.x * blockDim.x) {
    const int ab = (int)(i & 3);
    const int64_t co_ci = i >> 2;
    const int o = (int)(co_ci % co), c = (int)(co_ci / co);
    const T v = from_f<T>(w[i]);
    if (fwd) fwd[((int64_t)ab * co + o) * ci + c] = v;
    if (dgrad) dgrad[(int64_t)c * 4 * co + ab * co + o] = v;
  }
}

__global__ void unpack_conv3x3_kernel(const float* __restrict__ packed, int co, int ci, int ld, float* out) {
  const int64_t total = (int64_t)co * ci * 9;
  for (int64_t i = blockIdx.x * (int64_t)blockDim.x + threadIdx.x; i < total; i += (int64_t)gridDim.x * blockDim.x) {
    const int tap = (int)(i % 9);
    const int64_t oc = i / 9;
    const int c = (int)(oc % ci), o = (int)(oc / ci);
    out[i] = packed[(int64_t)o * ld + tap * ci + c];
  }
}

__global__ void unpack_convT_kernel(const float* __restrict__ packed, int ci, int co, int ld, float* out) {
  const int64_t total = (int64_t)ci * co * 4;
  for (int64_t i = blockIdx.x * (int64_t)blockDim.x + threadIdx.x; i < total; i += (int64_t)gridDim.x * blockDim.x) {
    const int ab = (int)(i & 3);
    const int64_t r = i >> 2;
    const int o = (int)(r % co), c = (int)(r / co);
    out[i] = packed[(int64_t)c * ld + ab * co + o];
  }
}

template <typename T>
__global__ void pack_weights_kernel(selunet_pack_list l, int64_t total) {
// ... 2102 lines not shown
```

### selectivenet_for_semantic_segmentation_binary_amd/engine.py

```python
from __future__ import annotations

import ctypes
import os
import weakref
from collections import OrderedDict
from dataclasses import dataclass, field

import torch

from . import _lib as K
from . import layout as LY

BN_EPS = 1e-5
BN_MOMENTUM = 0.1
BN_CENTER_RATIO = (None if os.environ.get("SELUNET_BN_TWOPASS", "0") == "1"
                   else float(os.environ.get("SELUNET_BN_FLAG_RATIO", "1.0")))
FIRST_KPAD = 32


X2_MODES = ("x2",)
EVAL_PATHS = ("exact", "split")


def _rup(a, b):
    return (a + b - 1) // b * b


def fp32_conv_path() -> str:
    if os.environ.get("SELUNET_X2", "1") != "0":
        return "split-fp16"
    return _exact_conv_path()


def _exact_conv_path() -> str:
    return "exact-fp32 (" + ("direct" if os.environ.get("SELUNET_WINO", "1") == "0" else "Winograd") + ")"


def check_eval_path(path) -> str:
    if path not in EVAL_PATHS:
        raise ValueError(f"fp32_eval_path {path!r}: one of {EVAL_PATHS}")
    return path


def fp32_eval_conv_path(eval_path="exact", compute_dtype=torch.float32) -> str:
    check_eval_path(eval_path)
    if compute_dtype != torch.float32:
        return "bf16"
    return fp32_conv_path() if eval_path == "split" else _exact_conv_path()


@dataclass
class BNState:
    y: torch.Tensor
    mean: torch.Tensor
    invstd: torch.Tensor
    scale: torch.Tensor
    shift: torch.Tensor
    n: int
    h: int
    w: int
    c: int
    amax: torch.Tensor = None
    name: str = ""

    def src(self):
        return K.source(self.y, self.c, self.scale, self.shift, relu=True, amax=self.amax)


@dataclass
class WPack:
    fwd: torch.Tensor
    dgrad: torch.Tensor
    kpad: int
    co: int
    mode: str = "direct"


@dataclass
class DGrad:
    t: torch.Tensor
    slab: torch.Tensor = None
    rows: int = 0
    apply: object = None
    da_word: bool = False
    src: object = None


def bnb_for(st: BNState, slab, amax=None) -> K.BnBwdStats:
    return K.BnBwdStats(K.ptr(st.y), K.ptr(st.scale), K.ptr(st.shift), K.ptr(st.mean), K.ptr(st.invstd), K.ptr(slab),
                        K.ptr(amax))


@dataclass
class Ctx:
    dt: torch.dtype
    training: bool
    selective: bool
    shape: tuple
    x: torch.Tensor = None
    entry: object = None
    bn: dict = field(default_factory=dict)
    pools: dict = field(default_factory=dict)
    ups: dict = field(default_factory=dict)
    wpack: dict = field(default_factory=dict)
    words: dict = field(default_factory=dict)
    x2: bool = False


class _Entry:

    def __init__(self, key):
        self.key = key
        self.plan = None
        self.ctx = None
        self.bwd = {}
        self.busy = False


class Engine:

    MAX_PLANS = 4

    def __init__(self, dt: torch.dtype = torch.float32):
        self.dt = dt
        self.code = K.dtype_code(dt)
        self.bke = 128 // torch.empty((), dtype=dt).element_size()
        self.plans_enabled = os.environ.get("SELUNET_NO_PLANS", "0") != "1"
        self.deterministic = os.environ.get("SELUNET_DETERMINISTIC", "1") != "0"
        self.x2 = dt == torch.float32 and os.environ.get("SELUNET_X2", "1") != "0"
        self.bn_shift = dt == torch.float32 and BN_CENTER_RATIO is not None and \
            os.environ.get("SELUNET_BN_SHIFT", "1") != "0"
        self.fuse_wgrad_apply = os.environ.get("SELUNET_FUSE_WGRAD_APPLY", "1") != "0"
        self.fuse_wgrad_src = os.environ.get("SELUNET_FUSE_WGRAD_SRC", "1") != "0"
        self._plans = OrderedDict()

    def _reduce(self, slab, rows, cols, out64=None, out32=None):
        ws = K.keep(torch.empty(K.query("selunet_reduce_ws_bytes", cols) // 8, dtype=torch.float64, device=slab.device))
        K.call("selunet_reduce_rows", K.ptr(slab), rows, cols, K.ptr(ws), K.ptr(out64), K.ptr(out32), self.stream)

    @property
    def stream(self):
        return K.stream_ptr()

    def _wgrad(self, gp, gq, packed):
        if not self.deterministic:
            K.call("selunet_memset", K.ptr(packed), 0, packed.numel() * 4, self.stream)
# ... 49 lines not shown
    def _shape_ok(self, query, name, ci, co, hw, need_dgrad):
        h, w = self._layer_hw(name, hw)
        ok = K.query(query, h, w, ci, self._concat_c0(name, ci), co) == 1
        return ok and (not need_dgrad or K.query(query, h, w, co, co, ci) == 1)

    def _wino_ok(self, name, ci, co, hw, need_dgrad):
        if self.dt != torch.float32 or hw is None or name == "encoder_layer_1_1":
            return False
        return self._shape_ok("selunet_conv3x3_wino_ok", name, ci, co, hw, need_dgrad)

    def _x2_ok(self, name, ci, co, hw, need_dgrad, training, eval_split=False):
        if not (self.x2 and (training or eval_split)) or hw is None or name == "encoder_layer_1_1":
            return False
        return self._shape_ok("selunet_conv3x3_x2_ok", name, ci, co, hw, need_dgrad)

    def pack_weights(self, P, need_dgrad=True, hw=None, training=False, heads=(), eval_split=False):
        dev = P["encoder_layer_1_2.0.weight"].device
        packs = {}
        pl = K.PackList()
        for name, ci, co in LY.CBR_LAYERS:
            w = P[f"{name}.0.weight"]
            ci = w.shape[1]
            dg = None
            if self._x2_ok(name, ci, co, hw, need_dgrad, training, eval_split):
                mode, kpad, kind = "x2", 9 * ci, K.PACK_CONV3X3_X2
                fwd = K.keep(torch.empty(co * kpad + co, dtype=torch.float32, device=dev))
                if need_dgrad:
                    dg = K.keep(torch.empty(ci * (kpad // ci) * co + ci, dtype=torch.float32, device=dev))
            else:
                if self._wino_ok(name, ci, co, hw, need_dgrad):
                    mode, kpad, taps, kind = "wino", 12 * ci, 12, K.PACK_CONV3X3_WINO
                else:
                    kpad = FIRST_KPAD if name == "encoder_layer_1_1" else _rup(9 * ci, self.bke)
                    mode, taps, kind = "direct", 9, K.PACK_CONV3X3
                fwd = K.keep(torch.empty(co, kpad, dtype=self.dt, device=dev))
                if need_dgrad and name != "encoder_layer_1_1":
                    dg = K.keep(torch.empty(ci, taps * co, dtype=self.dt, device=dev))
            pl.d[pl.n] = K.PackDesc(K.ptr(w), K.ptr(fwd), K.ptr(dg), kind, co, ci, kpad, 0)
            pl.n += 1
            packs[name] = WPack(fwd, dg, kpad, co, mode)
        x2 = any(wp.mode in X2_MODES for wp in packs.values())
        for name, ci, co in LY.UNPOOLS:
            w = P[f"{name}.weight"]
            if x2:
                fwd = K.keep(torch.empty(4 * co * ci + 4 * co, dtype=torch.float32, device=dev))
                dg = K.keep(torch.empty(ci * 4 * co + ci, dtype=torch.float32, device=dev)) if need_dgrad else None
                pl.d[pl.n] = K.PackDesc(K.ptr(w), K.ptr(fwd), K.ptr(dg), K.PACK_CONVT_X2, co, ci, ci, 0)
            else:
                fwd = K.keep(torch.empty(4 * co, ci, dtype=self.dt, device=dev))
                dg = K.keep(torch.empty(ci, 4 * co, dtype=self.dt, device=dev)) if need_dgrad else None
                pl.d[pl.n] = K.PackDesc(K.ptr(w), K.ptr(fwd), K.ptr(dg), K.PACK_CONVT, co, ci, 0, 0)
            pl.n += 1
            packs[name] = WPack(fwd, dg, ci, co, "x2" if x2 else "direct")
        if heads:
            no = sum(c for _, c in heads)
            hw_, hb_ = (K.keep(torch.empty(no, k, dtype=torch.float32, device=dev)) for k in (64, 1))
            k = 0
            if pl.n + 2 * len(heads) > K.PACK_MAX:
                raise ValueError(f"{len(heads)} heads: more weight-pack entries than SELUNET_PACK_MAX")
            for h, c in heads:
                for t, dst, n in ((P[f"{h}.weight"], hw_[k:], c * 64), (P[f"{h}.bias"], hb_[k:], c)):
                    pl.d[pl.n] = K.PackDesc(K.ptr(t), K.ptr(dst), None, K.PACK_COPY, n, 1, 0, 0)
                    pl.n += 1
                k += c
            packs["heads"] = (hw_, hb_.view(no))
        K.call("selunet_pack_weights", pl, self.code, self.stream)
        return packs

    def _word(self, ctx, key):
        return ctx.words[key]

    def _conv3x3(self, g, b, n_cols, kpad, ep, mode, srcs=()):
        if mode in X2_MODES:
            words = [s.amax for s in srcs]
            if any(wd is None for wd in words):
                raise RuntimeError("split-fp16 conv: a source without its range word")
            K.call("selunet_conv3x3_x2", g, K.ptr(b), n_cols, ep,
                   K.ptr(words[0]), K.ptr(words[1]) if len(words) > 1 else None, self.stream)
        elif mode == "wino":
            K.call("selunet_conv3x3_wino", g, K.ptr(b), n_cols, ep, self.stream)
        else:
            K.call("selunet_gemm_gather", g, K.ptr(b), n_cols, kpad, ep, self.code, self.stream)

    def _cbr(self, ctx, name, P, B, n, h, w, *srcs, taps=9, first_x=None):
        wp = ctx.wpack[name]
        fwd, kpad, co = wp.fwd, wp.kpad, wp.co
        M = n * h * w
        dev = fwd.device
        y = K.keep(torch.empty(M, co, dtype=self.dt, device=dev))
        stats = None
        if first_x is not None:
            rows = K.query("selunet_first_conv_rows", n, h, w)
        else:
            g = K.gather(n, h, w, taps, *srcs)
            rows = (K.query("selunet_conv3x3_x2_stats_rows", g, co) if wp.mode in X2_MODES
                    else K.query("selunet_gemm_stats_rows", g, co, self.code))
        center = None
        if ctx.training:
            stats = K.keep(torch.empty(rows, 2, co, dtype=torch.float32, device=dev))
            if self.bn_shift:
                center = K.keep(torch.zeros(co, dtype=torch.float32, device=dev))
        if first_x is not None:
            K.call("selunet_first_conv_fwd_centered", K.ptr(first_x), n, first_x.shape[1], h, w, K.ptr(fwd),
                   K.ptr(y), K.ptr(stats), K.ptr(center), self.code, self.stream)
        else:
            ep = K.Epilogue(K.ptr(y), None, None, K.ptr(stats), K.EP_PLAIN, 0)
            ep.stats_center = K.ptr(center)
            self._conv3x3(g, fwd, co, kpad, ep, wp.mode, srcs)
        mean, invstd, scale, shift = (K.keep(torch.empty(co, dtype=torch.float32, device=dev)) for _ in range(4))
        if ctx.training and self.dt == torch.float32:
            ws = K.keep(torch.empty(K.query("selunet_reduce_ws_bytes", 2 * co) // 8, dtype=torch.float64, device=dev))
            uvar = K.keep(torch.zeros(co, dtype=torch.float32, device=dev)) if BN_CENTER_RATIO is not None else None
            if center is not None:
                K.call("selunet_bn_stats_finalize_shifted", K.ptr(stats), rows, K.ptr(ws), M, co, K.ptr(center),
                       K.ptr(P[f"{name}.0.bias"]), K.ptr(P[f"{name}.1.weight"]), K.ptr(P[f"{name}.1.bias"]),
                       BN_CENTER_RATIO, K.ptr(mean), K.ptr(uvar), K.ptr(invstd), K.ptr(scale), K.ptr(shift),
                       self.stream)
            else:
                K.call("selunet_bn_stats_finalize", K.ptr(stats), rows, K.ptr(ws), None, M, co,
                       K.ptr(P[f"{name}.0.bias"]), K.ptr(P[f"{name}.1.weight"]), K.ptr(P[f"{name}.1.bias"]),
                       None, K.ptr(uvar), None, 1.0 if uvar is not None else BN_MOMENTUM, BN_EPS, K.ptr(mean),
                       K.ptr(invstd), K.ptr(scale), K.ptr(shift), self.stream)
            rows2 = K.query("selunet_bn_centered_rows", M)
            slab2 = K.keep(torch.empty(rows2, 2, co, dtype=torch.float32, device=dev))
            if uvar is not None:
                K.call("selunet_bn_centered_partials_adaptive", K.ptr(y), M, co, K.ptr(mean), K.ptr(uvar),
                       float("inf") if center is not None else BN_CENTER_RATIO, K.ptr(slab2), self.code,
                       self.stream)
            else:
                K.call("selunet_bn_centered_partials", K.ptr(y), M, co, K.ptr(mean), K.ptr(slab2), self.code,
                       self.stream)
            bound = self._word(ctx, "act:" + name) if ctx.x2 else None
            K.call("selunet_bn_stats_finalize_centered_bound", K.ptr(slab2), rows2, K.ptr(ws), None, M, co,
                   K.ptr(mean), K.ptr(P[f"{name}.0.bias"]), K.ptr(P[f"{name}.1.weight"]), K.ptr(P[f"{name}.1.bias"]),
                   K.ptr(B[f"{name}.1.running_mean"]), K.ptr(B[f"{name}.1.running_var"]),
                   K.ptr(B[f"{name}.1.num_batches_tracked"]), BN_MOMENTUM, BN_EPS,
                   K.ptr(mean), K.ptr(invstd), K.ptr(scale), K.ptr(shift), K.ptr(bound), self.stream)
        elif ctx.training:
            ws = K.keep(torch.empty(K.query("selunet_reduce_ws_bytes", 2 * co) // 8, dtype=torch.float64, device=dev))
            K.call("selunet_bn_stats_finalize", K.ptr(stats), rows, K.ptr(ws), None, M, co,
                   K.ptr(P[f"{name}.0.bias"]), K.ptr(P[f"{name}.1.weight"]), K.ptr(P[f"{name}.1.bias"]),
                   K.ptr(B[f"{name}.1.running_mean"]), K.ptr(B[f"{name}.1.running_var"]),
                   K.ptr(B[f"{name}.1.num_batches_tracked"]), BN_MOMENTUM, BN_EPS,
                   K.ptr(mean), K.ptr(invstd), K.ptr(scale), K.ptr(shift), self.stream)
        else:
            K.call("selunet_bn_finalize", None, M, co, K.ptr(P[f"{name}.0.bias"]), K.ptr(P[f"{name}.1.weight"]),
                   K.ptr(P[f"{name}.1.bias"]), K.ptr(B[f"{name}.1.running_mean"]), K.ptr(B[f"{name}.1.running_var"]),
                   K.ptr(B[f"{name}.1.num_batches_tracked"]), BN_MOMENTUM, BN_EPS, 0,
                   K.ptr(mean), K.ptr(invstd), K.ptr(scale), K.ptr(shift), self.stream)
        st = BNState(y, mean, invstd, scale, shift, n, h, w, co, name=name)
        if ctx.x2:
            st.amax = self._word(ctx, "act:" + name)
            if not ctx.training:
                K.call("selunet_act_amax", K.ptr(y), M, co, K.ptr(scale), K.ptr(shift), K.ptr(st.amax), self.stream)
            elif self.dt != torch.float32:
                K.call("selunet_act_bound", K.ptr(P[f"{name}.1.weight"]), K.ptr(P[f"{name}.1.bias"]), co, M,
                       K.ptr(st.amax), self.stream)
        ctx.bn[name] = st
        return st

    def _pool(self, ctx, key, st: BNState):
        out = K.keep(torch.empty(st.n * (st.h // 2) * (st.w // 2), st.c, dtype=self.dt, device=st.y.device))
        K.call("selunet_maxpool2_fwd", K.ptr(st.y), st.n, st.h, st.w, st.c, K.ptr(st.scale), K.ptr(st.shift),
               K.ptr(out), self.code, self.stream)
        ctx.pools[key] = out
        return out

    def _up(self, ctx, name, P, st: BNState):
        wp = ctx.wpack[name]
        fwd, ci, co = wp.fwd, wp.kpad, wp.co
        out = K.keep(torch.empty(st.n * 2 * st.h * 2 * st.w, co, dtype=self.dt, device=st.y.device))
        g = K.gather(st.n, st.h, st.w, 1, st.src())
        ep = K.Epilogue(K.ptr(out), None, K.ptr(P[f"{name}.bias"]), None, K.EP_SCATTER2X, 0)
        if ctx.x2:
            ep.amax = K.ptr(self._word(ctx, "up:" + name))
        if wp.mode == "x2":
            K.call("selunet_gemm_gather_x2", g, K.ptr(fwd), 4 * co, ci, ep, K.ptr(st.amax), None, self.stream)
        else:
            K.call("selunet_gemm_gather", g, K.ptr(fwd), 4 * co, ci, ep, self.code, self.stream)
        ctx.ups[name] = out
        return out

    def _signature(self, x, P, B, selective, training, need_backward):
        return (tuple(x.shape), x.device.index, bool(selective), bool(training), bool(need_backward), self.stream,
                tuple(t.data_ptr() for t in P.values()), tuple(t.data_ptr() for t in B.values()))

    def _entry_for(self, sig):
        lst = self._plans.get(sig)
        if lst is None:
            lst = self._plans[sig] = []
            while len(self._plans) > 2 * self.MAX_PLANS:
                for k, v in self._plans.items():
                    if k != sig and not any(e.busy for e in v):
                        del self._plans[k]
                        break
                else:
                    break
        self._plans.move_to_end(sig)
        for e in lst:
            if not e.busy:
                return e
        if len(lst) < self.MAX_PLANS:
            e = _Entry(sig)
            lst.append(e)
            return e
        return None

    @staticmethod
    def release(ctx):
        if ctx is not None and ctx.entry is not None:
            ctx.entry.busy = False

    def forward(self, x, P, B, selective, training, need_backward=False, ce_heads=None, eval_path="exact"):
        eval_split = check_eval_path(eval_path) == "split" and self.x2 and not training
        assert x.dim() == 4 and x.is_contiguous() and x.dtype == torch.float32
        n, cin, H, W = x.shape
        if H % 8 or W % 8:
            raise ValueError(f"UNet_B needs H and W divisible by 8 (three 2x2 poolings); got {H}x{W}")
        if ce_heads is None:
            nheads = 3 if selective else 1
            outs = tuple(torch.empty(n, H, W, dtype=torch.float32, device=x.device) for _ in range(nheads))
        else:
            ce_heads = tuple(ce_heads)
            outs = tuple(torch.empty(n, c, H, W, dtype=torch.float32, device=x.device) for _, c in ce_heads)
        e = self._entry_for(self._signature(x, P, B, selective, training, need_backward) + (ce_heads, eval_split)) \
            if self.plans_enabled else None
        slots = {"x": x, **{f"out{i}": o for i, o in enumerate(outs)}}
        if e is None:
            ctx = self._forward_impl(x, P, B, selective, training, need_backward, outs, ce_heads, eval_split)
        elif e.plan is not None:
            e.plan.replay(slots)
            ctx = e.ctx
            ctx.x = x
        else:
            plan = K.Plan(slots)
            with K.recording(plan):
                ctx = self._forward_impl(x, P, B, selective, training, need_backward, outs, ce_heads, eval_split)
            e.plan, e.ctx = plan, ctx
            ctx.entry = e
        if e is not None and training and need_backward:
            e.busy = True
        return outs, ctx

    def _forward_impl(self, x, P, B, selective, training, need_backward, outs, ce_heads=None, eval_split=False):
        n, cin, H, W = x.shape
        ctx = Ctx(self.dt, training, selective, (n, cin, H, W), x=x)
        ctx.ce_heads = ce_heads
        heads = LY.HEADS if selective else LY.HEADS[:1]
        heads = list(ce_heads) if ce_heads is not None else [(h, 1) for h in heads]
        if sum(c for _, c in heads) > 8:
            raise ValueError(f"the heads have {sum(c for _, c in heads)} output channels; the MI355X heads kernel "
                             "takes at most 8")
        ctx.wpack = self.pack_weights(P, need_dgrad=training and need_backward, hw=(H, W), training=training,
                                      heads=heads, eval_split=eval_split)
        hw, hb = ctx.wpack.pop("heads")
        ctx.x2 = any(wp.mode in X2_MODES for wp in ctx.wpack.values())
        if ctx.x2:
            keys = [f"{k}:{nm}" for nm, _, _ in LY.CBR_LAYERS for k in ("act", "dy", "du", "da", "dyb")]
            keys += ["up:" + nm for nm, _, _ in LY.UNPOOLS]
            buf = K.keep(torch.empty(len(keys), dtype=torch.float32, device=x.device))
            K.call("selunet_memset", K.ptr(buf), 0, buf.numel() * 4, self.stream)
            ctx.words = {k: buf[i:i + 1] for i, k in enumerate(keys)}
        c = lambda name, h, w, *s: self._cbr(ctx, name, P, B, n, h, w, *s)
        h1, w1, h2, w2, h3, w3, h4, w4 = H, W, H // 2, W // 2, H // 4, W // 4, H // 8, W // 8
        e11 = self._cbr(ctx, "encoder_layer_1_1", P, B, n, h1, w1, first_x=x)
        e12 = c("encoder_layer_1_2", h1, w1, e11.src())
        p1 = self._pool(ctx, "pool1", e12)
        wd = lambda st: st.amax
        e21 = c("encoder_layer_2_1", h2, w2, K.source(p1, 64, amax=wd(e12)))
        e22 = c("encoder_layer_2_2", h2, w2, e21.src())
        p2 = self._pool(ctx, "pool2", e22)
        e31 = c("encoder_layer_3_1", h3, w3, K.source(p2, 128, amax=wd(e22)))
        e32 = c("encoder_layer_3_2", h3, w3, e31.src())
        p3 = self._pool(ctx, "pool3", e32)
        b42 = c("decoder_layer_4_2", h4, w4, K.source(p3, 256, amax=wd(e32)))
        b41 = c("decoder_layer_4_1", h4, w4, b42.src())
        u3 = self._up(ctx, "unpool3", P, b41)
        uw = lambda nm: ctx.words.get("up:" + nm)
        d32 = c("decoder_layer_3_2", h3, w3, K.source(u3, 256, amax=uw("unpool3")), e32.src())
        d31 = c("decoder_layer_3_1", h3, w3, d32.src())
        u2 = self._up(ctx, "unpool2", P, d31)
        d22 = c("decoder_layer_2_2", h2, w2, K.source(u2, 128, amax=uw("unpool2")), e22.src())
        d21 = c("decoder_layer_2_1", h2, w2, d22.src())
        u1 = self._up(ctx, "unpool1", P, d21)
        d12 = c("decoder_layer_1_2", h1, w1, K.source(u1, 64, amax=uw("unpool1")), e12.src())
        d11 = c("decoder_layer_1_1", h1, w1, d12.src())
        M = n * H * W
        if ce_heads is not None:
            return self._heads_fwd_planes(ctx, d11, outs, ce_heads, n, H * W, hw, hb)
        o = list(outs) + [None] * (3 - len(outs))
        K.call("selunet_heads_fwd", K.ptr(d11.y), M, K.ptr(d11.scale), K.ptr(d11.shift), K.ptr(hw), K.ptr(hb),
               len(heads), K.ptr(o[0]), K.ptr(o[1]), K.ptr(o[2]), self.code, self.stream)
        ctx.head_w = hw
        return ctx

    @staticmethod
    def _planes(tensors, ce_heads, hw, with_slab=False):
        d = K.HeadPlanes()
        k, off = 0, 0
        for t, (_, c) in zip(tensors, ce_heads):
            for j in range(c):
                d.plane[k] = t.data_ptr() + j * hw * 4
                d.img_stride[k] = c * hw
                d.w_off[k] = off + j * 64
                d.b_off[k] = off + c * 64 + j
                k += 1
            off += c * 65
        d.n, d.hw, d.row_len = k, hw, off
        return d

    def _heads_fwd_planes(self, ctx, d11, outs, ce_heads, n, hw, w, b):
        K.call("selunet_heads_fwd_planes", K.ptr(d11.y), n * hw, K.ptr(d11.scale), K.ptr(d11.shift), K.ptr(w), K.ptr(b),
               self._planes(outs, ce_heads, hw), self.code, self.stream)
        ctx.head_w = w
        return ctx

    def _cbr_bwd(self, ctx, name, dg: DGrad, G, input_srcs, dgrad_split=None, need_dgrad=True, q_taps=9,
                 prev: BNState = None, first_x=None):
        st: BNState = ctx.bn[name]
        M, co, dev = st.n * st.h * st.w, st.c, st.y.device
        coef = K.keep(torch.empty(3, co, dtype=torch.float32, device=dev))
        gamma = ctx.params[f"{name}.1.weight"]
        ws = K.keep(torch.empty(K.query("selunet_reduce_ws_bytes", 3 * co) // 8, dtype=torch.float64, device=dev))
        wp = ctx.wpack[name] if first_x is None else None
        ci = sum(s.channels for s in input_srcs)
        src = dg.src if (dg.src is not None and co == 64 and self.fuse_wgrad_src) else None
        fuse = (wp is not None and wp.mode in X2_MODES and dg.da_word and self.fuse_wgrad_apply and
                (src is not None or (dg.apply is None and dg.t is not None)) and
                all(sr.amax is not None for sr in input_srcs))
        gp = gq = None
        if fuse:
            gp = K.gather(st.n, st.h, st.w, 1, K.source(dg.t if src is None else st.y, co))
            gq = K.gather(st.n, st.h, st.w, q_taps, *input_srcs)
            fuse = K.query("selunet_conv3x3_wgrad_x2_ws_bytes", gp, gq) > 0
        if fuse:
            K.call("selunet_bn_bwd_stats_finalize_bound", K.ptr(dg.slab), dg.rows, K.ptr(ws), None, M, co, K.ptr(gamma),
                   K.ptr(st.invstd), K.ptr(G[f"{name}.1.weight"]), K.ptr(G[f"{name}.1.bias"]),
                   K.ptr(G[f"{name}.0.bias"]), K.ptr(coef), K.ptr(self._word(ctx, "da:" + name)),
                   K.ptr(self._word(ctx, "dyb:" + name)), self.stream)
        else:
            K.call("selunet_bn_bwd_stats_finalize", K.ptr(dg.slab), dg.rows, K.ptr(ws), None, M, co, K.ptr(gamma),
                   K.ptr(st.invstd), K.ptr(G[f"{name}.1.weight"]), K.ptr(G[f"{name}.1.bias"]),
                   K.ptr(G[f"{name}.0.bias"]), K.ptr(coef), self.stream)
        if first_x is not None:
            cin = first_x.shape[1]
            rows = K.query("selunet_first_conv_wgrad_rows", st.n, st.h, st.w)
            slab = K.keep(torch.empty(rows, co, FIRST_KPAD, dtype=torch.float32, device=dev))
            K.call("selunet_first_conv_wgrad_bn", K.ptr(first_x), st.n, cin, st.h, st.w, K.ptr(dg.t), K.ptr(st.y),
                   K.ptr(st.scale), K.ptr(st.shift), K.ptr(st.mean), K.ptr(st.invstd), K.ptr(coef), K.ptr(slab),
                   self.code, self.stream)
            packed = K.keep(torch.empty(co, FIRST_KPAD, dtype=torch.float32, device=dev))
            self._reduce(slab, rows, co * FIRST_KPAD, out32=packed)
            K.call("selunet_unpack_conv3x3_grad", K.ptr(packed), co, cin, FIRST_KPAD, K.ptr(G[f"{name}.0.weight"]),
                   self.stream)
            K.marker(("grads", name))
            return None
        dy = K.keep(torch.empty(M, co, dtype=self.dt, device=dev))
        dyw = self._word(ctx, "dy:" + name) if wp.mode in X2_MODES else None
# ... 131 lines not shown
    def _backward_impl(self, ctx, P, G, g_heads):
        ctx.params = P
        n, cin, H, W = ctx.shape
        M = n * H * W
        dev = ctx.x.device
        bn = ctx.bn
        heads = LY.HEADS if ctx.selective else LY.HEADS[:1]
        d11 = bn["decoder_layer_1_1"]
        rows = K.query("selunet_channel_slab_rows", M)
        bslab = K.keep(torch.empty(rows, 3, 64, dtype=torch.float32, device=dev))
        ce = getattr(ctx, "ce_heads", None)
        if ce is not None:
            heads = [h for h, _ in ce]
            gs = [g if g is not None else K.keep(torch.zeros(n, c, H, W, dtype=torch.float32, device=dev))
                  for g, (_, c) in zip(g_heads, ce)]
            planes = self._planes(gs, ce, H * W, with_slab=True)
            slab = K.keep(torch.empty(rows, planes.row_len, dtype=torch.float32, device=dev))
            fused = K.fused_apply_enabled()
            dz = None if fused else K.keep(torch.empty(M, 64, dtype=self.dt, device=dev))
            K.call("selunet_heads_bwd_planes", K.ptr(d11.y), M, K.ptr(d11.scale), K.ptr(d11.shift), K.ptr(ctx.head_w),
                   planes, K.ptr(dz), K.ptr(slab), bnb_for(d11, bslab), self.code, self.stream)
            seg = planes.row_len
            head_w = ctx.head_w

            def apply_planes(dy, coef, word):
                K.call("selunet_bn_bwd_apply_heads_planes", K.ptr(d11.y), M, K.ptr(d11.scale), K.ptr(d11.shift),
                       K.ptr(d11.mean), K.ptr(d11.invstd), K.ptr(coef), K.ptr(head_w), planes, K.ptr(dy),
                       K.ptr(word), self.code, self.stream)
        else:
            gs = [g if g is not None else K.keep(torch.zeros(n, H, W, dtype=torch.float32, device=dev))
                  for g in g_heads]
            gs = gs + [None] * (3 - len(gs))
            nh = len(heads)
            slab = K.keep(torch.empty(rows, nh * 65, dtype=torch.float32, device=dev))
            fused = K.fused_apply_enabled()
            dz = None if fused else K.keep(torch.empty(M, 64, dtype=self.dt, device=dev))
            hword = ctx.words.get("da:decoder_layer_1_1") if (ctx.x2 and fused) else None
            K.call("selunet_heads_bwd", K.ptr(d11.y), M, K.ptr(d11.scale), K.ptr(d11.shift), K.ptr(ctx.head_w), nh,
                   K.ptr(gs[0]), K.ptr(gs[1]), K.ptr(gs[2]), K.ptr(dz), K.ptr(slab), bnb_for(d11, bslab, hword),
                   self.code, self.stream)
            seg = nh * 65
        apply = apply_planes if (ce is not None and dz is None) else None
        hsrc = None
        if dz is None and ce is None:
            head_w = ctx.head_w

            def apply(dy, coef, word):
                K.call("selunet_bn_bwd_apply_heads", K.ptr(d11.y), M, K.ptr(d11.scale), K.ptr(d11.shift),
                       K.ptr(d11.mean), K.ptr(d11.invstd), K.ptr(coef), K.ptr(head_w), nh, K.ptr(gs[0]), K.ptr(gs[1]),
                       K.ptr(gs[2]), K.ptr(dy), K.ptr(word), self.code, self.stream)
            g3 = (ctypes.c_void_p * 3)(*[K.ptr(g) for g in gs[:3]])
            hsrc = K.DaSource(K.DA_HEADS, nh, None, None, K.ptr(head_w), g3)
        dz = DGrad(dz, bslab, rows, apply, da_word=hsrc is not None and hword is not None, src=hsrc)
        hw0 = G[f"{heads[0]}.weight"]
        off = 0
        for h in heads:
            assert G[f"{h}.weight"].data_ptr() == hw0.data_ptr() + off * 4
            off += G[f"{h}.weight"].numel()
            assert G[f"{h}.bias"].data_ptr() == hw0.data_ptr() + off * 4
            off += G[f"{h}.bias"].numel()
        assert off == seg
        self._reduce(slab, rows, seg, out32=hw0)
        K.marker(("grads", "heads"))

        e12, e22, e32 = bn["encoder_layer_1_2"], bn["encoder_layer_2_2"], bn["encoder_layer_3_2"]
        u1, u2, u3 = ctx.ups["unpool1"], ctx.ups["unpool2"], ctx.ups["unpool3"]
        p1, p2, p3 = ctx.pools["pool1"], ctx.pools["pool2"], ctx.pools["pool3"]
        cb = lambda name, d, srcs, **kw: self._cbr_bwd(ctx, name, d, G, srcs, **kw)
        uw = lambda nm: ctx.words.get("up:" + nm)

        dz = cb("decoder_layer_1_1", dz, [bn["decoder_layer_1_2"].src()], prev=bn["decoder_layer_1_2"])
        du1, dskip1 = cb("decoder_layer_1_2", dz, [K.source(u1, 64, amax=uw("unpool1")), e12.src()],
                            dgrad_split=64)
        dz = self._up_bwd(ctx, "unpool1", du1, G, bn["decoder_layer_2_1"])
        dz = cb("decoder_layer_2_1", dz, [bn["decoder_layer_2_2"].src()], prev=bn["decoder_layer_2_2"])
        du2, dskip2 = cb("decoder_layer_2_2", dz, [K.source(u2, 128, amax=uw("unpool2")), e22.src()],
                            dgrad_split=128)
        dz = self._up_bwd(ctx, "unpool2", du2, G, bn["decoder_layer_3_1"])
        dz = cb("decoder_layer_3_1", dz, [bn["decoder_layer_3_2"].src()], prev=bn["decoder_layer_3_2"])
        du3, dskip3 = cb("decoder_layer_3_2", dz, [K.source(u3, 256, amax=uw("unpool3")), e32.src()],
                            dgrad_split=256)
        dz = self._up_bwd(ctx, "unpool3", du3, G, bn["decoder_layer_4_1"])
        dz = cb("decoder_layer_4_1", dz, [bn["decoder_layer_4_2"].src()], prev=bn["decoder_layer_4_2"])
        dp3 = cb("decoder_layer_4_2", dz, [K.source(p3, 256, amax=e32.amax)])
        dz = self._pool_bwd(ctx, e32, dp3, dskip3)
        dz = cb("encoder_layer_3_2", dz, [bn["encoder_layer_3_1"].src()], prev=bn["encoder_layer_3_1"])
        dp2 = cb("encoder_layer_3_1", dz, [K.source(p2, 128, amax=e22.amax)])
        dz = self._pool_bwd(ctx, e22, dp2, dskip2)
        dz = cb("encoder_layer_2_2", dz, [bn["encoder_layer_2_1"].src()], prev=bn["encoder_layer_2_1"])
        dp1 = cb("encoder_layer_2_1", dz, [K.source(p1, 64, amax=e12.amax)])
        dz = self._pool_bwd(ctx, e12, dp1, dskip1)
        dz = cb("encoder_layer_1_2", dz, [bn["encoder_layer_1_1"].src()], prev=bn["encoder_layer_1_1"])
        cb("encoder_layer_1_1", dz, [], need_dgrad=False, first_x=ctx.x)
```

Baseline: 1452 images/s.

## Fold 2x2 max-pool of raw conv output into conv3x3 epilogue using BN sign

The split-fp16 conv3x3 kernels (persistent halo and x2d) now also write a 2x2-pooled output from the LDS tile in their epilogue. Because BN scale followed by ReLU is monotone per channel, the kernel picks max or min of the raw window according to the sign of the BN gamma. The downstream pool source then applies scale/shift/relu lazily, so the three encoder maxpool launches and their full-resolution activation re-reads are skipped. In exchange the epilogue grows, and correctness depends on scale having the same sign as gamma (positive invstd).

```diff
diff --git a/include/selunet.h b/include/selunet.h
--- a/include/selunet.h
+++ b/include/selunet.h
@@ -33,6 +33,7 @@
   SELUNET_OPT_TILE_QUEUE,
   SELUNET_OPT_X2P,
   SELUNET_OPT_CONVT_RING,
+  SELUNET_OPT_POOL_FOLD,
   SELUNET_OPT_COUNT
 };
 int64_t selunet_set_option(int32_t key, int64_t value);
@@ -80,6 +81,8 @@
   selunet_bn_bwd_stats bnb;
   float* amax;
   const float* stats_center;
+  float* pool;
+  const float* pool_sign;
 } selunet_epilogue;
 
 const char* selunet_last_error(void);
@@ -129,6 +132,7 @@
                                     float* out, const float* amax_p, const float* amax_q0, const float* amax_q1,
                                     const selunet_bn_bwd_stats* bnb, const float* coef, const selunet_da_source* src,
                                     float* dy, float* dy_amax, void* stream);
+int32_t selunet_conv3x3_x2_pool_ok(const selunet_gather* a, int32_t n_cols);
 int selunet_conv3x3_x2(const selunet_gather* a, const float* w, int32_t n_cols, const selunet_epilogue* ep,
                        const float* amax0, const float* amax1, void* stream);
 const char* selunet_conv3x3_x2_kernel_name(const selunet_gather* a, int32_t n_cols, int32_t mode, int32_t split);
diff --git a/selectivenet_for_semantic_segmentation_binary_amd/_lib.py b/selectivenet_for_semantic_segmentation_binary_amd/_lib.py
--- a/selectivenet_for_semantic_segmentation_binary_amd/_lib.py
+++ b/selectivenet_for_semantic_segmentation_binary_amd/_lib.py
@@ -43,7 +43,7 @@
 class Epilogue(ctypes.Structure):
     _fields_ = [("out0", c_void_p), ("out1", c_void_p), ("bias", c_void_p), ("stats", c_void_p),
                 ("mode", c_int32), ("split", c_int32), ("colsum", c_void_p), ("bnb", BnBwdStats),
-                ("amax", c_void_p), ("stats_center", c_void_p)]
+                ("amax", c_void_p), ("stats_center", c_void_p), ("pool", c_void_p), ("pool_sign", c_void_p)]
 
 
 class PackDesc(ctypes.Structure):
@@ -95,6 +95,7 @@
     "selunet_conv3x3_x2": (c_int32, [ctypes.POINTER(Gather), P, c_int32, ctypes.POINTER(Epilogue), P, P, P]),
     "selunet_conv3x3_x2_kernel_name": (ctypes.c_char_p, [ctypes.POINTER(Gather), c_int32, c_int32, c_int32]),
     "selunet_conv3x3_x2_stats_rows": (c_int64, [ctypes.POINTER(Gather), c_int32]),
+    "selunet_conv3x3_x2_pool_ok": (c_int32, [ctypes.POINTER(Gather), c_int32]),
     "selunet_act_bound": (c_int32, [P, P, c_int32, c_int64, P, P]),
     "selunet_act_amax": (c_int32, [P, c_int64, c_int32, P, P, P, P]),
     "selunet_conv3x3_wgrad_x2_ws_bytes": (c_int64, [ctypes.POINTER(Gather), ctypes.POINTER(Gather)]),
@@ -259,7 +260,7 @@
 OPT = {name: i for i, name in enumerate([
     "HALO", "HALO_PERSIST", "WINO", "WINO_WGRAD", "WINO_WGRAD_TW", "WINO_WGRAD_WAVES", "WGRAD_WGS",
     "X2_WGRAD_WGS", "GEMM_WGRAD_WGS", "GATHER_WGS", "RF_SINGLE", "APPLY_U8", "APPLY_GRID", "X2D",
-    "TILE_QUEUE", "X2P", "CONVT_RING"])}
+    "TILE_QUEUE", "X2P", "CONVT_RING", "POOL_FOLD"])}
 ENV_OPTIONS = {f"SELUNET_{k}": v for k, v in OPT.items() if k != "HALO"}
 
 
diff --git a/selectivenet_for_semantic_segmentation_binary_amd/csrc/conv3x3.hip b/selectivenet_for_semantic_segmentation_binary_amd/csrc/conv3x3.hip
--- a/selectivenet_for_semantic_segmentation_binary_amd/csrc/conv3x3.hip
+++ b/selectivenet_for_semantic_segmentation_binary_amd/csrc/conv3x3.hip
@@ -239,7 +239,7 @@
   lds_tile_store<T, TH * TW, BN, HTHREADS>(tile, tid, dst, ep.bias, bias_col, tile_stats(ep, ptile, n0, N));
 }
 
-template <typename T, int BN, bool X2, bool M16 = false, bool TQ = false>
+template <typename T, int BN, bool X2, bool M16 = false, bool TQ = false, bool POOL = false>
 __global__ void __launch_bounds__(HTHREADS, 1)
 conv3x3_halo_persist_kernel(GatherArg g, const T* __restrict__ B, int N, int k_pad, EpiArg ep, int n_tiles,
                             int tiles_x, int tiles_y, int ptiles, int gp, const float* __restrict__ wcs,
@@ -247,6 +247,7 @@
                             unsigned* __restrict__ tq = nullptr) {
   static_assert(!TQ || X2, "tile queue: split-fp16 kernel only");
   static_assert(!X2 || std::is_same<T, float>::value, "split-fp16 form of fp32 operands only");
+  static_assert(!POOL || (X2 && !TQ), "pooled output: split-fp16 kernel, static walk");
   static_assert(!M16 || X2, "16x16x32 form: split-fp16 only (the bf16 form lost every A/B, retired in round 6)");
   constexpr int E = 16 / sizeof(T);
   constexpr int CK = 128 / sizeof(T);
@@ -781,6 +782,8 @@
       return reinterpret_cast<T*>(ep.out0) + m * N + col;
     };
     auto bias_col = [&](int cl) { return n0 + cl; };
+    unsigned psb = 0;
+    if constexpr (POOL) psb = pool_sign_bits<BN>(ep.pool_sign + n0, tid);
     if constexpr (TQ) {
       TileStats tt = tile_stats(ep, pt_cur, n0, N);
       lds_tile_store_acc<T, TH * TW, BN, HTHREADS>(tile, tid, dst, ep.bias, bias_col, tt, s1, s2, s3, amx);
@@ -790,6 +793,15 @@
       for (int e = 0; e < 8; ++e) s1[e] = s2[e] = s3[e] = 0;
     } else {
       lds_tile_store_acc<T, TH * TW, BN, HTHREADS>(tile, tid, dst, ep.bias, bias_col, ts, s1, s2, s3, amx);
+    }
+    if constexpr (POOL) {
+      auto pdst = [&](int wy, int wx, int cl) -> float* {
+        const int y = y0 + 2 * wy, x = x0 + 2 * wx;
+        if (y >= g.h || x >= g.w) return nullptr;
+        const int64_t m = ((int64_t)img * (g.h >> 1) + (y >> 1)) * (g.w >> 1) + (x >> 1);
+        return ep.pool + m * N + n0 + cl;
+      };
+      lds_tile_pool_store<BN, HTHREADS>(tile, tid, psb, pdst);
     }
     if (TQ ? pt_next < ptiles : i + 1 < ntl) {
       __syncthreads();
@@ -2474,8 +2486,11 @@
       return fail(SELUNET_ELAUNCH, "conv3x3_x2: tile-queue counters unavailable (set SELUNET_OPT_TILE_QUEUE "
                                    "before capturing the step)");
   }
-  auto k = tq ? conv3x3_halo_persist_kernel<float, BN, true, BN == 64, true>
-              : conv3x3_halo_persist_kernel<float, BN, true, BN == 64>;
+  if (tq != nullptr && ep.pool != nullptr)
+    return fail(SELUNET_EINVAL, "conv3x3_x2: the tile-queue form writes no pooled output");
+  auto k = tq        ? conv3x3_halo_persist_kernel<float, BN, true, BN == 64, true>
+           : ep.pool ? conv3x3_halo_persist_kernel<float, BN, true, BN == 64, false, true>
+                     : conv3x3_halo_persist_kernel<float, BN, true, BN == 64>;
   hipLaunchKernelGGL(k, dim3((unsigned)(gp * n_tiles)), dim3(HTHREADS), 0, st, g, w, N, k_pad, ep, n_tiles, tiles_x,
                      tiles_y, (int)conv3x3_halo_tiles(g), gp, w + (int64_t)N * k_pad, amax0, amax1, tq);
   return 0;
diff --git a/selectivenet_for_semantic_segmentation_binary_amd/csrc/conv3x3_x2d.hip b/selectivenet_for_semantic_segmentation_binary_amd/csrc/conv3x3_x2d.hip
--- a/selectivenet_for_semantic_segmentation_binary_amd/csrc/conv3x3_x2d.hip
+++ b/selectivenet_for_semantic_segmentation_binary_amd/csrc/conv3x3_x2d.hip
@@ -11,6 +11,7 @@
 constexpr int XD_A_ROUNDS = (XD_HPIX * 8 + XD_THREADS - 1) / XD_THREADS;
 constexpr int XD_B_ROUNDS = XD_BN * 8 / XD_THREADS;
 
+template <bool POOL>
 __global__ void __launch_bounds__(XD_THREADS, 2)
 conv3x3_x2d_kernel(GatherArg g, const float* __restrict__ B, int k_pad, EpiArg ep, int tiles_x, int tiles_y,
                    int ptiles, int gp, const float* __restrict__ wcs, const float* __restrict__ amax0,
@@ -316,7 +317,18 @@
       return reinterpret_cast<float*>(ep.out0) + m * N + cl;
     };
     auto bias_col = [&](int cl) { return cl; };
+    unsigned psb = 0;
+    if constexpr (POOL) psb = pool_sign_bits<N>(ep.pool_sign, tid);
     lds_tile_store_acc<float, XD_TH * XD_TW, N, XD_THREADS>(tile, tid, dst, ep.bias, bias_col, ts, s1, s2, s3, amx);
+    if constexpr (POOL) {
+      auto pdst = [&](int wy, int wx, int cl) -> float* {
+        const int y = y0 + 2 * wy, x = x0 + 2 * wx;
+        if (y >= g.h || x >= g.w) return nullptr;
+        const int64_t m = ((int64_t)img * (g.h >> 1) + (y >> 1)) * (g.w >> 1) + (x >> 1);
+        return ep.pool + m * N + cl;
+      };
+      lds_tile_pool_store<N, XD_THREADS>(tile, tid, psb, pdst);
+    }
     if (i + 1 < ntl) {
       __syncthreads();
       a_store(ra);
@@ -351,8 +363,9 @@
       (int64_t)((XD_TH + 2) * g.w + XD_HW) * cmax * 4 >= (int64_t)1 << 31 || (int64_t)16 * g.w + XD_HW >= 1 << 24 ||
       (int64_t)cmax * 4 >= 1 << 24 || (int64_t)k_pad * 4 >= 1 << 24)
     return fail(SELUNET_EINVAL, "conv3x3_x2d: operand too large for 32-bit staging offsets");
-  hipLaunchKernelGGL(conv3x3_x2d_kernel, dim3((unsigned)gp), dim3(XD_THREADS), 0, st, g, w, k_pad, ep, tiles_x, tiles_y,
-                     ptiles, gp, w + (int64_t)XD_BN * k_pad, amax0, amax1);
+  auto k = ep.pool ? conv3x3_x2d_kernel<true> : conv3x3_x2d_kernel<false>;
+  hipLaunchKernelGGL(k, dim3((unsigned)gp), dim3(XD_THREADS), 0, st, g, w, k_pad, ep, tiles_x, tiles_y, ptiles, gp,
+                     w + (int64_t)XD_BN * k_pad, amax0, amax1);
   return check_launch("conv3x3_x2d");
 }
 
diff --git a/selectivenet_for_semantic_segmentation_binary_amd/csrc/gemm.hip b/selectivenet_for_semantic_segmentation_binary_amd/csrc/gemm.hip
--- a/selectivenet_for_semantic_segmentation_binary_amd/csrc/gemm.hip
+++ b/selectivenet_for_semantic_segmentation_binary_amd/csrc/gemm.hip
@@ -989,7 +989,8 @@
 }
 
 static int check_gather_call(const selunet_gather* a, const void* b, int32_t n_cols, int32_t k_pad,
-                             const selunet_epilogue* ep, int32_t dtype, GatherArg& g, EpiArg& e) {
+                             const selunet_epilogue* ep, int32_t dtype, GatherArg& g, EpiArg& e,
+                             bool allow_pool = false) {
   SELUNET_REQUIRE(dtype == SELUNET_F32 || dtype == SELUNET_BF16, "dtype must be SELUNET_F32 or SELUNET_BF16");
   const int esz = dtype == SELUNET_F32 ? 4 : 2;
   const int bke = 128 / esz;
@@ -1016,6 +1017,15 @@
   e = EpiArg{ep->out0, ep->out1, ep->bias, ep->stats, ep->mode, ep->split, ep->colsum,
              BnBwdArg{bb.y, bb.scale, bb.shift, bb.mean, bb.invstd, bb.slab}, ep->amax, ep->stats_center};
   SELUNET_REQUIRE(ep->stats_center == nullptr || ep->stats != nullptr, "stats_center only with stats");
+  if (ep->pool != nullptr) {
+    SELUNET_REQUIRE(allow_pool, "epilogue.pool: only selunet_conv3x3_x2 writes a pooled output");
+    SELUNET_REQUIRE(ep->mode == SELUNET_EP_PLAIN && ep->pool_sign != nullptr && dtype == SELUNET_F32 &&
+                        ep->bias == nullptr,
+                    "epilogue.pool needs the plain fp32 epilogue without bias, and pool_sign");
+    SELUNET_REQUIRE(a->h % 2 == 0 && a->w % 2 == 0, "epilogue.pool: H and W must be even (got %d x %d)", a->h, a->w);
+    e.pool = ep->pool;
+    e.pool_sign = ep->pool_sign;
+  }
   return SELUNET_OK;
 }
 
@@ -1146,14 +1156,28 @@
   return conv3x3_x2_persist_rows(g, n_cols);
 }
 
+static bool x2_writes_pool(const GatherArg& g, int n_cols) {
+  return g.h % 2 == 0 && g.w % 2 == 0 &&
+         (conv3x3_x2d_eligible(g, n_cols) || (!conv3x3_x2p_eligible(g, n_cols) && !x2_tile_queue()));
+}
+
+extern "C" int32_t selunet_conv3x3_x2_pool_ok(const selunet_gather* a, int32_t n_cols) {
+  GatherArg g;
+  if (option(SELUNET_OPT_POOL_FOLD, 1) == 0 || a == nullptr || a->taps != 9 || make_gather(a, SELUNET_F32, g, 4))
+    return 0;
+  return halo_enabled() && conv3x3_x2_eligible(g, n_cols) && x2_writes_pool(g, n_cols) ? 1 : 0;
+}
+
 extern "C" int selunet_conv3x3_x2(const selunet_gather* a, const float* w, int32_t n_cols, const selunet_epilogue* ep,
                                   const float* amax0, const float* amax1, void* stream) {
   GatherArg g;
   EpiArg e;
   SELUNET_REQUIRE(a != nullptr && a->taps == 9, "conv3x3_x2: a 3x3 (taps = 9) gather is required");
   if (int rc = check_gather_call(a, w, n_cols, 9 * (a->src[0].channels + (a->nsrc > 1 ? a->src[1].channels : 0)), ep,
-                                 SELUNET_F32, g, e))
+                                 SELUNET_F32, g, e, true))
     return rc;
+  SELUNET_REQUIRE(e.pool == nullptr || x2_writes_pool(g, n_cols),
+                  "conv3x3_x2: the kernel of this operand writes no pooled output (see selunet_conv3x3_x2_pool_ok)");
   SELUNET_REQUIRE(ep->mode != SELUNET_EP_SCATTER2X, "conv3x3_x2: scatter epilogue not supported");
   SELUNET_REQUIRE(amax0 != nullptr && (a->nsrc == 1 || amax1 != nullptr),
                   "conv3x3_x2: every source needs its range word (amax0, amax1)");
diff --git a/selectivenet_for_semantic_segmentation_binary_amd/csrc/gemm_common.h b/selectivenet_for_semantic_segmentation_binary_amd/csrc/gemm_common.h
--- a/selectivenet_for_semantic_segmentation_binary_amd/csrc/gemm_common.h
+++ b/selectivenet_for_semantic_segmentation_binary_amd/csrc/gemm_common.h
@@ -162,6 +162,8 @@
   BnBwdArg bnb;
   float* amax;
   const float* stats_center;
+  float* pool;
+  const float* pool_sign;
 };
 
 typedef short s16x4 __attribute__((ext_vector_type(4)));
@@ -377,6 +379,41 @@
   float am = 0.0f;
   lds_tile_store_acc<T, TR, TC, NTHREADS>(tile, tid, dst, bias, bias_col, ts, s1, s2, s3, am);
   tile_stats_flush<TC, NTHREADS>(tile, tid, ts, s1, s2, s3, am);
+}
+
+template <int TC>
+__device__ __forceinline__ unsigned pool_sign_bits(const float* sign, int tid) {
+  const int col = (tid % (TC / 4)) * 4;
+  unsigned b = 0;
+#pragma unroll
+  for (int e = 0; e < 4; ++e) b |= (sign[col + e] >= 0.0f ? 1u : 0u) << e;
+  return b;
+}
+
+template <int TC, int NTHREADS, typename PDst>
+__device__ __forceinline__ void lds_tile_pool_store(const float* tile, int tid, unsigned sbits, PDst&& pdst) {
+  constexpr int CQ = TC / 4;
+  constexpr int WS = NTHREADS / CQ;
+  constexpr int LD = TC + 4;
+  static_assert(NTHREADS % CQ == 0 && 64 % WS == 0, "pool windows must split evenly over the threads");
+  const int col = (tid % CQ) * 4;
+#pragma unroll 1
+  for (int wi = tid / CQ; wi < 64; wi += WS) {
+    const int wy = wi >> 3, wx = wi & 7;
+    float* p = pdst(wy, wx, col);
+    if (p == nullptr) continue;
+    const float* t = tile + (wy * 32 + wx * 2) * LD + col;
+    const f32x4 a = *reinterpret_cast<const f32x4*>(t), b = *reinterpret_cast<const f32x4*>(t + LD);
+    const f32x4 c = *reinterpret_cast<const f32x4*>(t + 16 * LD), d = *reinterpret_cast<const f32x4*>(t + 17 * LD);
+    f32x4 o;
+#pragma unroll
+    for (int e = 0; e < 4; ++e) {
+      const float hi = fmaxf(fmaxf(a[e], b[e]), fmaxf(c[e], d[e]));
+      const float lo = fminf(fminf(a[e], b[e]), fminf(c[e], d[e]));
+      o[e] = (sbits >> e & 1u) ? hi : lo;
+    }
+    *reinterpret_cast<f32x4*>(p) = o;
+  }
 }
 
 int make_gather(const selunet_gather* a, int dtype, GatherArg& g, int vec_elems);
diff --git a/selectivenet_for_semantic_segmentation_binary_amd/csrc/pointwise.hip b/selectivenet_for_semantic_segmentation_binary_amd/csrc/pointwise.hip
--- a/selectivenet_for_semantic_segmentation_binary_amd/csrc/pointwise.hip
+++ b/selectivenet_for_semantic_segmentation_binary_amd/csrc/pointwise.hip
@@ -8,8 +8,8 @@
 
 static thread_local char g_err[512] = "";
 
-int64_t g_options[SELUNET_OPT_COUNT] = {-1, -1, -1, -1, -1, -1, -1, -1, -1, -1, -1, -1, -1, -1, -1, -1, -1};
-static_assert(SELUNET_OPT_COUNT == 17, "g_options initialiser: one -1 per option");
+int64_t g_options[SELUNET_OPT_COUNT] = {-1, -1, -1, -1, -1, -1, -1, -1, -1, -1, -1, -1, -1, -1, -1, -1, -1, -1};
+static_assert(SELUNET_OPT_COUNT == 18, "g_options initialiser: one -1 per option");
 
 void set_error(const char* fmt, ...) {
   va_list ap;
diff --git a/selectivenet_for_semantic_segmentation_binary_amd/engine.py b/selectivenet_for_semantic_segmentation_binary_amd/engine.py
--- a/selectivenet_for_semantic_segmentation_binary_amd/engine.py
+++ b/selectivenet_for_semantic_segmentation_binary_amd/engine.py
@@ -62,6 +62,7 @@
     c: int
     amax: torch.Tensor = None
     name: str = ""
+    pooled: torch.Tensor = None
 
     def src(self):
         return K.source(self.y, self.c, self.scale, self.shift, relu=True, amax=self.amax)
@@ -277,13 +278,13 @@
         else:
             K.call("selunet_gemm_gather", g, K.ptr(b), n_cols, kpad, ep, self.code, self.stream)
 
-    def _cbr(self, ctx, name, P, B, n, h, w, *srcs, taps=9, first_x=None):
+    def _cbr(self, ctx, name, P, B, n, h, w, *srcs, taps=9, first_x=None, pooled=False):
         wp = ctx.wpack[name]
         fwd, kpad, co = wp.fwd, wp.kpad, wp.co
         M = n * h * w
         dev = fwd.device
         y = K.keep(torch.empty(M, co, dtype=self.dt, device=dev))
-        stats = None
+        stats = praw = None
         if first_x is not None:
             rows = K.query("selunet_first_conv_rows", n, h, w)
         else:
@@ -301,6 +302,10 @@
         else:
             ep = K.Epilogue(K.ptr(y), None, None, K.ptr(stats), K.EP_PLAIN, 0)
             ep.stats_center = K.ptr(center)
+            if (pooled and ctx.training and self.dt == torch.float32 and wp.mode in X2_MODES
+                    and K.query("selunet_conv3x3_x2_pool_ok", g, co)):
+                praw = K.keep(torch.empty(n * (h // 2) * (w // 2), co, dtype=self.dt, device=dev))
+                ep.pool, ep.pool_sign = K.ptr(praw), K.ptr(P[f"{name}.1.weight"])
             self._conv3x3(g, fwd, co, kpad, ep, wp.mode, srcs)
         mean, invstd, scale, shift = (K.keep(torch.empty(co, dtype=torch.float32, device=dev)) for _ in range(4))
         if ctx.training and self.dt == torch.float32:
@@ -343,7 +348,7 @@
                    K.ptr(P[f"{name}.1.bias"]), K.ptr(B[f"{name}.1.running_mean"]), K.ptr(B[f"{name}.1.running_var"]),
                    K.ptr(B[f"{name}.1.num_batches_tracked"]), BN_MOMENTUM, BN_EPS, 0,
                    K.ptr(mean), K.ptr(invstd), K.ptr(scale), K.ptr(shift), self.stream)
-        st = BNState(y, mean, invstd, scale, shift, n, h, w, co, name=name)
+        st = BNState(y, mean, invstd, scale, shift, n, h, w, co, name=name, pooled=praw)
         if ctx.x2:
             st.amax = self._word(ctx, "act:" + name)
             if not ctx.training:
@@ -355,11 +360,16 @@
         return st
 
     def _pool(self, ctx, key, st: BNState):
+        if st.pooled is not None:
+            src = K.source(st.pooled, st.c, st.scale, st.shift, relu=True, amax=st.amax)
+            ctx.pools[key] = src
+            return src
         out = K.keep(torch.empty(st.n * (st.h // 2) * (st.w // 2), st.c, dtype=self.dt, device=st.y.device))
         K.call("selunet_maxpool2_fwd", K.ptr(st.y), st.n, st.h, st.w, st.c, K.ptr(st.scale), K.ptr(st.shift),
                K.ptr(out), self.code, self.stream)
-        ctx.pools[key] = out
-        return out
+        src = ctx.pools[key] = K.source(out, st.c, amax=st.amax)
+        src.tensor = out
+        return src
 
     def _up(self, ctx, name, P, st: BNState):
         wp = ctx.wpack[name]
@@ -456,19 +466,18 @@
             buf = K.keep(torch.empty(len(keys), dtype=torch.float32, device=x.device))
             K.call("selunet_memset", K.ptr(buf), 0, buf.numel() * 4, self.stream)
             ctx.words = {k: buf[i:i + 1] for i, k in enumerate(keys)}
-        c = lambda name, h, w, *s: self._cbr(ctx, name, P, B, n, h, w, *s)
+        c = lambda name, h, w, *s, **kw: self._cbr(ctx, name, P, B, n, h, w, *s, **kw)
         h1, w1, h2, w2, h3, w3, h4, w4 = H, W, H // 2, W // 2, H // 4, W // 4, H // 8, W // 8
         e11 = self._cbr(ctx, "encoder_layer_1_1", P, B, n, h1, w1, first_x=x)
-        e12 = c("encoder_layer_1_2", h1, w1, e11.src())
+        e12 = c("encoder_layer_1_2", h1, w1, e11.src(), pooled=True)
         p1 = self._pool(ctx, "pool1", e12)
-        wd = lambda st: st.amax
-        e21 = c("encoder_layer_2_1", h2, w2, K.source(p1, 64, amax=wd(e12)))
-        e22 = c("encoder_layer_2_2", h2, w2, e21.src())
+        e21 = c("encoder_layer_2_1", h2, w2, p1)
+        e22 = c("encoder_layer_2_2", h2, w2, e21.src(), pooled=True)
         p2 = self._pool(ctx, "pool2", e22)
-        e31 = c("encoder_layer_3_1", h3, w3, K.source(p2, 128, amax=wd(e22)))
-        e32 = c("encoder_layer_3_2", h3, w3, e31.src())
+        e31 = c("encoder_layer_3_1", h3, w3, p2)
+        e32 = c("encoder_layer_3_2", h3, w3, e31.src(), pooled=True)
         p3 = self._pool(ctx, "pool3", e32)
-        b42 = c("decoder_layer_4_2", h4, w4, K.source(p3, 256, amax=wd(e32)))
+        b42 = c("decoder_layer_4_2", h4, w4, p3)
         b41 = c("decoder_layer_4_1", h4, w4, b42.src())
         u3 = self._up(ctx, "unpool3", P, b41)
         uw = lambda nm: ctx.words.get("up:" + nm)
@@ -766,13 +775,13 @@
                             dgrad_split=256)
         dz = self._up_bwd(ctx, "unpool3", du3, G, bn["decoder_layer_4_1"])
         dz = cb("decoder_layer_4_1", dz, [bn["decoder_layer_4_2"].src()], prev=bn["decoder_layer_4_2"])
-        dp3 = cb("decoder_layer_4_2", dz, [K.source(p3, 256, amax=e32.amax)])
+        dp3 = cb("decoder_layer_4_2", dz, [p3])
         dz = self._pool_bwd(ctx, e32, dp3, dskip3)
         dz = cb("encoder_layer_3_2", dz, [bn["encoder_layer_3_1"].src()], prev=bn["encoder_layer_3_1"])
-        dp2 = cb("encoder_layer_3_1", dz, [K.source(p2, 128, amax=e22.amax)])
+        dp2 = cb("encoder_layer_3_1", dz, [p2])
         dz = self._pool_bwd(ctx, e22, dp2, dskip2)
         dz = cb("encoder_layer_2_2", dz, [bn["encoder_layer_2_1"].src()], prev=bn["encoder_layer_2_1"])
-        dp1 = cb("encoder_layer_2_1", dz, [K.source(p1, 64, amax=e12.amax)])
+        dp1 = cb("encoder_layer_2_1", dz, [p1])
         dz = self._pool_bwd(ctx, e12, dp1, dskip1)
         dz = cb("encoder_layer_1_2", dz, [bn["encoder_layer_1_1"].src()], prev=bn["encoder_layer_1_1"])
         cb("encoder_layer_1_1", dz, [], need_dgrad=False, first_x=ctx.x)
```

Result: no change. 1458 images/s (median of 6 runs) (+0.4%).
